# toposware/certificate-stark

Measured on AMD Instinct MI355X. Metric: proofs/sec, state_transition AIR @ 2^20 steps (complete prove(): trace gen, LDE, Blake3 commitments, constraint evaluation, composition, DEEP, FRI, 96 queries), higher is better.
Workload: dtype u64 (63-bit prime field, Montgomery) + u32 (Blake3)

## Files before the change

### certificate-stark_amd/backend.py

```python
import ctypes as C

import numpy as np
import torch

from . import _lib
from ._lib import check, u64p, u8p


def _np_u64(a):
    return np.ascontiguousarray(a, dtype=np.uint64)


def to_numpy_u64(t):
    return t.detach().cpu().contiguous().numpy().view(np.uint64)


class ProofBatch:

    def __init__(self, buf, stride, lens):
        self._buf, self._stride, self._lens = buf, stride, lens

    def __len__(self):
        return len(self._lens)

# ... 22 lines not shown
        self.device = torch.device("cuda", torch.cuda.current_device() if device is None else device)
        torch.cuda.set_device(self.device)
        self.stream = torch.cuda.current_stream(self.device)
        ctx = C.c_void_p()
        check(self.lib.cstark_ctx_create(C.c_int(self.device.index), C.c_void_p(self.stream.cuda_stream), C.byref(ctx)))
        self.ctx = ctx
        self.n_tx = 0
        self.depth = 0
        self.resident = None

    def close(self):
        if getattr(self, "ctx", None):
            self.lib.cstark_ctx_destroy(self.ctx)
            self.ctx = None

    def __del__(self):
        try:
            self.close()
        except Exception:
            pass

    def synchronize(self):
        check(self.lib.cstark_ctx_synchronize(self.ctx))

    def empty_u64(self, *shape):
        return torch.empty(shape, dtype=torch.int64, device=self.device)

    def from_numpy_u64(self, a):
        return torch.from_numpy(_np_u64(a).view(np.int64)).to(self.device)

    @staticmethod
    def _ptr(t, typ=u64p):
        assert t.is_contiguous()
        return C.cast(C.c_void_p(t.data_ptr()), typ)

    def upload_witness(self, w):
        self.resident = None
        s = _lib.TxWitnessStruct()
        s.n_tx, s.merkle_depth = int(w.n_tx), int(w.depth)
        keep = []
        for f, typ in (("initial_roots", u64p), ("final_root", u64p), ("s_old_values", u64p), ("r_old_values", u64p),
                       ("s_indices", u64p), ("r_indices", u64p), ("s_paths", u64p), ("r_paths", u64p),
                       ("deltas", u64p), ("sig_rx", u64p), ("sig_s", u8p)):
            a = np.ascontiguousarray(getattr(w, f), dtype=np.uint8 if typ is u8p else np.uint64)
            keep.append(a)
            setattr(s, f, a.ctypes.data_as(typ))
        check(self.lib.cstark_tx_witness_upload(self.ctx, C.byref(s)))
        self.n_tx, self.depth = int(w.n_tx), int(w.depth)

    def build_trace(self, out=None):
        n = self.n_tx * _lib.TX_CYCLE_LENGTH
        if out is None:
            out = self.empty_u64(_lib.TX_TRACE_WIDTH, n)
        assert out.shape == (_lib.TX_TRACE_WIDTH, n) and out.dtype == torch.int64
        check(self.lib.cstark_tx_build_trace(self.ctx, self._ptr(out)))
        return out

    def field_generator(self):
        self.lib.cstark_field_generator.restype = C.c_uint64
        return int(self.lib.cstark_field_generator())

    def field_lde_offset(self):
        self.lib.cstark_field_lde_offset.restype = C.c_uint64
        return int(self.lib.cstark_field_lde_offset())

    def interpolate_columns(self, evals, out=None):
        width, n = evals.shape
        if out is None:
            out = self.empty_u64(width, n)
        check(self.lib.cstark_interpolate_columns(self.ctx, self._ptr(evals), self._ptr(out), C.c_uint32(width),
                                                  C.c_uint32(n.bit_length() - 1)))
        return out

    def lde_columns(self, coeffs, log_blowup, offset=None, k0=0, nk=None, out=None):
        width, n = coeffs.shape
        nk = (1 << log_blowup) - k0 if nk is None else nk
        if out is None:
            out = self.empty_u64(nk, width, n)
        off = self.field_lde_offset() if offset is None else int(offset)
        check(self.lib.cstark_lde_columns(self.ctx, self._ptr(coeffs), self._ptr(out), C.c_uint32(width),
                                          C.c_uint32(n.bit_length() - 1), C.c_uint32(log_blowup), C.c_uint64(off),
                                          C.c_uint32(k0), C.c_uint32(nk)))
        return out

    def empty_u8(self, *shape):
        return torch.empty(shape, dtype=torch.uint8, device=self.device)

    def hash_rows_fn(self, hash_fn, lde, log_blowup, k0=0):
        nk, width, n = lde.shape
        leaves = self.empty_u8(n << log_blowup, 32)
        check(self.lib.cstark_hash_rows_fn(self.ctx, C.c_uint32(hash_fn), self._ptr(lde), self._ptr(leaves, u8p), C.c_uint32(width),
                                           C.c_uint32(n.bit_length() - 1), C.c_uint32(log_blowup), C.c_uint32(k0), C.c_uint32(nk)))
        return leaves

    def merkle_build_fn(self, hash_fn, nodes):
        check(self.lib.cstark_merkle_build_fn(self.ctx, C.c_uint32(hash_fn), self._ptr(nodes, u8p), C.c_uint32((nodes.shape[0] // 2).bit_length() - 1)))
        return nodes

    def hash_rows(self, lde, log_blowup, k0=0, leaves=None):
        nk, width, n = lde.shape
        if leaves is None:
            leaves = torch.zeros((n << log_blowup, 32), dtype=torch.uint8, device=self.device)
        check(self.lib.cstark_hash_rows(self.ctx, self._ptr(lde), self._ptr(leaves, u8p), C.c_uint32(width),
                                        C.c_uint32(n.bit_length() - 1), C.c_uint32(log_blowup), C.c_uint32(k0), C.c_uint32(nk)))
        return leaves

    def merkle_build(self, nodes):
        L2 = nodes.shape[0]
        check(self.lib.cstark_merkle_build(self.ctx, self._ptr(nodes, u8p), C.c_uint32((L2 // 2).bit_length() - 1)))
        return nodes

    def evaluate_transitions(self, lde, depth, log_blowup=3, k0=0):
        nk, width, n = lde.shape
        out = self.empty_u64(nk, _lib.TX_NUM_CONSTRAINTS, n)
        check(self.lib.cstark_tx_evaluate_transitions(self.ctx, self._ptr(lde), self._ptr(out), C.c_uint32(depth),
                                                      C.c_uint32(n.bit_length() - 1), C.c_uint32(log_blowup), C.c_uint32(k0), C.c_uint32(nk)))
        return out

    def evaluate_constraints(self, lde, coeffs, pub_inputs, depth, log_blowup=3, k0=0, out=None, input_is_lde=False):
        nk, width, n = lde.shape
        if out is None:
            out = self.empty_u64(nk, n)
        pub = (C.c_uint64 * 4)(*[int(v) for v in pub_inputs])
        if input_is_lde:
            assert k0 == 0 and nk == 8 and log_blowup == 3
            check(self.lib.cstark_tx_evaluate_constraints_lde(self.ctx, self._ptr(lde), C.byref(coeffs), pub, self._ptr(out), C.c_uint32(depth),
                                                              C.c_uint32(n.bit_length() - 1)))
            return out
        check(self.lib.cstark_tx_evaluate_constraints(self.ctx, self._ptr(lde), C.byref(coeffs), pub, self._ptr(out), C.c_uint32(depth),
                                                      C.c_uint32(n.bit_length() - 1), C.c_uint32(log_blowup), C.c_uint32(k0), C.c_uint32(nk)))
        return out

    def evaluate_constraints_ext(self, lde, coeff_sets, pub_inputs, depth, log_blowup=3, k0=0, input_is_lde=False):
        nk, width, n = lde.shape
        m = len(coeff_sets)
        out = self.empty_u64(m, nk, n)
        arr = (type(coeff_sets[0]) * m)(*coeff_sets)
        pub = (C.c_uint64 * 4)(*[int(v) for v in pub_inputs])
        if input_is_lde:
            assert k0 == 0 and nk == 8 and log_blowup == 3
            check(self.lib.cstark_tx_evaluate_constraints_ext_lde(self.ctx, self._ptr(lde), arr, C.c_uint32(m), pub, self._ptr(out),
                                                                  C.c_uint32(depth), C.c_uint32(n.bit_length() - 1)))
            return out
        check(self.lib.cstark_tx_evaluate_constraints_ext(self.ctx, self._ptr(lde), arr, C.c_uint32(m), pub, self._ptr(out), C.c_uint32(depth),
                                                          C.c_uint32(n.bit_length() - 1), C.c_uint32(log_blowup), C.c_uint32(k0), C.c_uint32(nk)))
        return out

    AIR_TRANSACTION, AIR_MERKLE, AIR_SCHNORR, AIR_RANGE, AIR_RESCUE_CHAIN = 0, 1, 2, 3, 4

    def rescue_chain_build_trace(self, seed, chain_length):
        s = _np_u64(seed)
        out = self.empty_u64(14, 8 * chain_length)
        check(self.lib.cstark_rescue_chain_build_trace(self.ctx, self._hptr(s), C.c_uint32(chain_length), self._ptr(out)))
        return out

    def rescue_prove(self, options, seed, chain_length):
        s = _np_u64(seed)
        o = self._options_struct(options)
        self.lib.cstark_tx_proof_size_bound.restype = C.c_size_t
        cap = 2 * self.lib.cstark_tx_proof_size_bound(C.c_uint32(max(1, chain_length // 128)), C.byref(o))
        buf = (C.c_uint8 * cap)()
        n = C.c_size_t(0)
        check(self.lib.cstark_rescue_prove(self.ctx, C.byref(o), self._hptr(s), C.c_uint32(chain_length), buf, C.c_size_t(cap), C.byref(n)))
        return bytes(memoryview(buf)[:n.value])

    def merkle_build_trace(self):
# ... 379 lines not shown
```

### certificate-stark_amd/csrc/capi.hip

```cpp
#include <hip/hip_runtime.h>
#include <stdio.h>
#include <stdlib.h>
#include <string.h>
#include <deque>
#include <new>
#include <vector>
#include "../../include/cstark.h"
#include "air_tx_host.h"
#include "blake3.h"
#include "ctx.h"
#include "constraints.h"
#include "deep.h"
#include "ext.h"
#include "hostfield.h"
#include "ntt.h"
#include "trace_gen.h"

namespace cs { thread_local char g_err[512] = ""; }
using cs::fail;
using cs::NttPlan;
using cs::CosetTable;
using cs::PeriodicTable;
using cs::g_err;

// ... 37 lines not shown
    return CSTARK_OK;
}

int get_coset_table(cstark_ctx *c, unsigned log_n, unsigned log_b, uint64_t offset, const CosetTable **out) {
    for (const CosetTable &t : c->cosets)
        if (t.log_n == log_n && t.log_b == log_b && t.offset == offset) { *out = &t; return CSTARK_OK; }
    const size_t n = (size_t)1 << log_n, b = (size_t)1 << log_b;
    CosetTable t{log_n, log_b, offset, nullptr};
    DevGuard g;
    HIP_TRY(g.alloc(&t.s, b * n * 8));
    const uint64_t wbn = cs::host::root_of_unity(log_n + log_b);
    uint64_t shift = offset;
    for (size_t k = 0; k < b; k++) {
        HIP_TRY(cs::ntt_power_table(t.s + k * n, n, shift, c->stream));
        shift = cs::host::mul(shift, wbn);
    }
    cs::NttThreeStepShape shape;
    if (cs::ntt_three_step_shape(log_n, &shape)) {
        const NttPlan *p;
        RC_TRY(get_plan(c, log_n, &p));
        t.aux_words = cs::ntt_aux_coset_words(shape);
        HIP_TRY(g.alloc(&t.aux, b * t.aux_words * 8));
        for (size_t k = 0; k < b; k++) HIP_TRY(cs::ntt_build_aux_coset(t.aux + k * t.aux_words, p->w, t.s + k * n, shape, c->stream));
    }
    c->cosets.push_back(t);
    g.release();
    *out = &c->cosets.back();
    return CSTARK_OK;
}

int ensure_ws(cstark_ctx *c, size_t bytes) {
    if (bytes <= c->ws_bytes) return CSTARK_OK;
    if (c->ws) { HIP_TRY(hipStreamSynchronize(c->stream)); HIP_TRY(hipFree(c->ws)); c->ws = nullptr; c->ws_bytes = 0; }
    HIP_TRY(hipMalloc(&c->ws, bytes));
    c->ws_bytes = bytes;
    return CSTARK_OK;
}

}
int plan_tables(cstark_ctx *c, unsigned log_n, const uint64_t **w, const uint64_t **winv) {
    const NttPlan *p;
    RC_TRY(get_plan(c, log_n, &p));
    *w = p->w; *winv = p->winv;
    return CSTARK_OK;
}
namespace {

int interpolate_impl(cstark_ctx *c, uint64_t *d_evals, uint64_t *d_coeffs, uint32_t width, uint32_t log_n) {
    if (!c || !d_evals || !d_coeffs || width == 0) return fail(CSTARK_ERR_INVALID_ARG, "cstark_interpolate_columns: bad argument");
    if (d_evals == d_coeffs) return fail(CSTARK_ERR_INVALID_ARG, "cstark_interpolate_columns: output must not alias input");
    if (log_n < cs::NTT_MIN_LOG_N || log_n > cs::NTT_MAX_LOG_N) return fail(CSTARK_ERR_UNSUPPORTED, "domain size must be 2^6 .. 2^24");
    HIP_TRY(hipSetDevice(c->device));
    const NttPlan *p;
    RC_TRY(get_plan(c, log_n, &p));
    cs::NttArgs a{};
    a.in = d_evals; a.scratch = d_evals; a.out = d_coeffs;
    a.width = width; a.batch = 1; a.log_n = log_n;
    a.w = p->winv; a.post_scale = p->n_inv; a.do_scale = true; a.inverse = true; a.aux = p->aux_winv;
    HIP_TRY(cs::ntt_columns(a, c->stream));
    return CSTARK_OK;
}

constexpr size_t LDE_EVENT_CAP = 4096;
int lde_mark(cstark_ctx *c) {
    if (c->lde_ev_used == c->lde_ev.size()) {
        if (c->lde_ev.size() >= LDE_EVENT_CAP) return CSTARK_ERR_UNSUPPORTED;

        hipEvent_t e;
        HIP_TRY(hipEventCreate(&e));
        c->lde_ev.push_back(e);
    }
    HIP_TRY(hipEventRecord(c->lde_ev[c->lde_ev_used++], c->stream));
    return CSTARK_OK;
}

const size_t LDE_BATCH_WS_BYTES = [] {
    const char *e = getenv("CSTARK_LDE_BATCH_MB");
    if (!e) return (size_t)7 << 30;
    const long long mb = atoll(e);
    return mb <= 0 ? (size_t)0 : mb > (64ll << 10) ? (size_t)64 << 30 : (size_t)mb << 20;
}();
int lde_impl_inner(cstark_ctx *c, const uint64_t *d_coeffs, uint64_t *d_lde, uint32_t width, uint32_t col0, uint32_t ncols, uint32_t log_n,
                   uint32_t log_blowup, uint64_t domain_offset, uint32_t k0, uint32_t nk);
int lde_impl(cstark_ctx *c, const uint64_t *d_coeffs, uint64_t *d_lde, uint32_t width, uint32_t col0, uint32_t ncols, uint32_t log_n, uint32_t log_blowup,
             uint64_t domain_offset, uint32_t k0, uint32_t nk) {
    bool timed = c && c->part_timing && c->lde_ev_used + 2 <= LDE_EVENT_CAP;
    const size_t mark = timed ? c->lde_ev_used : 0;
    if (timed && lde_mark(c) != CSTARK_OK) { c->lde_ev_used = mark; timed = false; }
    const int rc = lde_impl_inner(c, d_coeffs, d_lde, width, col0, ncols, log_n, log_blowup, domain_offset, k0, nk);
    if (timed) {
        if (rc == CSTARK_OK && lde_mark(c) == CSTARK_OK) c->lde_units += (uint64_t)ncols * nk << log_n;
        else c->lde_ev_used = mark;
    }
    return rc;
}
int lde_impl_inner(cstark_ctx *c, const uint64_t *d_coeffs, uint64_t *d_lde, uint32_t width, uint32_t col0, uint32_t ncols, uint32_t log_n,
                   uint32_t log_blowup, uint64_t domain_offset, uint32_t k0, uint32_t nk) {
    if (!c || !d_coeffs || !d_lde || width == 0 || ncols == 0 || (uint64_t)col0 + ncols > width) return fail(CSTARK_ERR_INVALID_ARG, "cstark_lde_columns: bad argument");
    if (log_n < cs::NTT_MIN_LOG_N || log_n > cs::NTT_MAX_LOG_N || log_blowup > 6) return fail(CSTARK_ERR_UNSUPPORTED, "unsupported domain size");
    if (domain_offset == 0 || domain_offset >= cs::host::P) return fail(CSTARK_ERR_INVALID_ARG, "domain offset must be a nonzero field element");
    if ((uint64_t)k0 + nk > (1ull << log_blowup)) return fail(CSTARK_ERR_INVALID_ARG, "coset range exceeds the blowup factor");
    HIP_TRY(hipSetDevice(c->device));
    const NttPlan *p;
    const CosetTable *t;
    RC_TRY(get_plan(c, log_n, &p));
    RC_TRY(get_coset_table(c, log_n, log_blowup, domain_offset, &t));
    const size_t n = (size_t)1 << log_n;
    RC_TRY(ensure_ws(c, (size_t)width * n * 8));
    cs::NttArgs a{};
    a.in = d_coeffs + (size_t)col0 * n; a.scratch = (uint64_t *)c->ws;
    a.width = ncols; a.log_n = log_n;
    a.w = p->w; a.do_scale = false; a.aux = p->aux_w;
    if (nk > 1 && (size_t)nk * ncols * n * 8 <= LDE_BATCH_WS_BYTES) {
        if (ensure_ws(c, (size_t)nk * ncols * n * 8) == CSTARK_OK) {
            a.scratch = (uint64_t *)c->ws; a.out = d_lde + (size_t)col0 * n; a.batch = nk;
            a.prescale = t->s + (size_t)k0 * n; a.prescale_batch_stride = n;
            a.aux_ps = t->aux ? t->aux + (size_t)k0 * t->aux_words : nullptr; a.aux_ps_batch_stride = t->aux_words;
            a.in_batch_stride = 0; a.scratch_batch_stride = (size_t)ncols * n; a.out_batch_stride = (size_t)width * n;
            HIP_TRY(cs::ntt_columns(a, c->stream));
            return CSTARK_OK;
        }
        (void)hipGetLastError();
        RC_TRY(ensure_ws(c, (size_t)width * n * 8));
        a.scratch = (uint64_t *)c->ws;
    }
    a.batch = 1;
    for (uint32_t k = k0; k < k0 + nk; k++) {
        a.out = d_lde + ((size_t)(k - k0) * width + col0) * n;
        a.prescale = t->s + (size_t)k * n;
        a.aux_ps = t->aux ? t->aux + (size_t)k * t->aux_words : nullptr;
        HIP_TRY(cs::ntt_columns(a, c->stream));
    }
    return CSTARK_OK;
}

int extend_periodic_columns(cstark_ctx *c, const std::vector<uint64_t> &cols, uint32_t ncols, uint32_t log_cycle, unsigned log_n, unsigned log_b,
                            DevGuard &keep, uint64_t **d_tab) {
    const size_t words = (size_t)ncols << log_cycle, n = (size_t)1 << log_n;
    uint64_t *d_cols = nullptr, *d_poly = nullptr;
    DevGuard tmp;
    HIP_TRY(tmp.alloc(&d_cols, words * 8));
    HIP_TRY(tmp.alloc(&d_poly, words * 8));
    HIP_TRY(keep.alloc(d_tab, (words << log_b) * 8));
    HIP_TRY(hipMemcpyAsync(d_cols, cols.data(), words * 8, hipMemcpyHostToDevice, c->stream));
    RC_TRY(interpolate_impl(c, d_cols, d_poly, ncols, log_cycle));
    RC_TRY(lde_impl(c, d_poly, *d_tab, ncols, 0, ncols, log_cycle, log_b, cs::host::pow(cs::host::lde_offset(), n >> log_cycle), 0, 1u << log_b));
    HIP_TRY(hipStreamSynchronize(c->stream));
    return CSTARK_OK;
}

int get_periodic(cstark_ctx *c, unsigned depth, unsigned log_n, unsigned log_b, const PeriodicTable **out) {
    for (const PeriodicTable &t : c->periodic)
        if (t.depth == depth && t.log_n == log_n && t.log_b == log_b) { *out = &t; return CSTARK_OK; }
    if (log_n < 10) return fail(CSTARK_ERR_INVALID_ARG, "the trace must hold at least one 1024-row transaction");
    std::vector<uint64_t> cols;
    if (!cs::host::tx_periodic_columns(depth, cols)) return fail(CSTARK_ERR_INVALID_ARG, "unsupported Merkle depth");
    static_assert(cs::host::TX_CYCLE == 1 << 10, "the cycle of TransactionAir's periodic columns");
    const size_t n = (size_t)1 << log_n, b = (size_t)1 << log_b;
    PeriodicTable t{depth, log_n, log_b, nullptr, nullptr, nullptr};
    DevGuard keep;
    RC_TRY(extend_periodic_columns(c, cols, cs::host::TX_NUM_PERIODIC, 10, log_n, log_b, keep, &t.tab));
    HIP_TRY(keep.alloc(&t.coset, b * cs::CE_COSET_CONSTS * 8));
    const uint64_t g = cs::host::lde_offset();
    std::vector<uint64_t> cc(b * cs::CE_COSET_CONSTS);
    const uint64_t wbn = cs::host::root_of_unity(log_n + log_b);
    uint64_t shift = g;
    for (size_t k = 0; k < b; k++) {
        uint64_t *o = cc.data() + k * cs::CE_COSET_CONSTS;
        o[0] = shift;
        o[1] = cs::host::inv(cs::host::sub(cs::host::pow(shift, n), cs::host::ONE));
        for (int gi = 0; gi < 5; gi++) o[2 + gi] = cs::host::pow(shift, cs::host::tx_group_adjustment(gi, n, n * b));
        o[7] = cs::host::pow(shift, cs::host::tx_boundary_adjustment(n, n * b));
        o[8] = cs::host::pow(shift, n - 1);
        o[9] = 0;
        shift = cs::host::mul(shift, wbn);
    }
    HIP_TRY(hipMemcpyAsync(t.coset, cc.data(), cc.size() * 8, hipMemcpyHostToDevice, c->stream));
    const NttPlan *plan;
    RC_TRY(get_plan(c, log_n, &plan));
    HIP_TRY(keep.alloc(&t.binv, b * 2 * n * 8));
    HIP_TRY(cs::build_boundary_inverses(t.binv, plan->w, t.coset, cs::host::inv(cs::host::root_of_unity(log_n)), log_n, log_b, c->stream));
    HIP_TRY(hipStreamSynchronize(c->stream));
    keep.release();
    c->periodic.push_back(t);
    *out = &c->periodic.back();
    return CSTARK_OK;
}

int get_small_periodic(cstark_ctx *c, int air, unsigned depth, unsigned log_n, unsigned log_b, const PeriodicTable **out) {
    for (const PeriodicTable &t : c->small_periodic)
        if (t.air == air && t.depth == depth && t.log_n == log_n && t.log_b == log_b) { *out = &t; return CSTARK_OK; }
    PeriodicTable t{depth, log_n, log_b, nullptr, nullptr, nullptr, air};
    std::vector<uint64_t> cols;
    DevGuard keep;
    if (air == CSTARK_AIR_MERKLE_UPDATE) {
        if (!cs::host::merkle_periodic_columns(depth, cols)) return fail(CSTARK_ERR_INVALID_ARG, "unsupported Merkle depth");
        RC_TRY(extend_periodic_columns(c, cols, 33, 9, log_n, log_b, keep, &t.tab));
    } else if (air == CSTARK_AIR_SCHNORR) {
        cs::host::schnorr_mask_columns(cols);
        RC_TRY(extend_periodic_columns(c, cols, 36, 9, log_n, log_b, keep, &t.tab));
    } else if (air == CSTARK_AIR_RESCUE_CHAIN) {
        using namespace cs::host;
        rescue_chain_periodic_columns(cols);
        const size_t n = (size_t)1 << log_n, b = (size_t)1 << log_b;
        for (int cidx = 0; cidx < 29; cidx++) intt_small(cols.data() + (size_t)cidx * 8, 3);
        std::vector<uint64_t> tab(b * 29 * 8);
        const uint64_t wbn = root_of_unity(log_n + log_b), w8 = root_of_unity(3);
        uint64_t shift = lde_offset();
        for (size_t k = 0; k < b; k++) {
            uint64_t x = pow(shift, n / 8);
            for (int m = 0; m < 8; m++) {
                for (int cidx = 0; cidx < 29; cidx++) {
                    const uint64_t *co = cols.data() + (size_t)cidx * 8;
                    uint64_t v = 0;
                    for (int d = 7; d >= 0; d--) v = add(mul(v, x), co[d]);
                    tab[(k * 29 + cidx) * 8 + m] = v;
// ... 18 lines not shown
              uint32_t nk, cs::CeParams *p) {
    if (!c || !d_lde || !d_out) return fail(CSTARK_ERR_INVALID_ARG, "constraint evaluation: null argument");
    if (((uintptr_t)d_lde & 15) != 0) return fail(CSTARK_ERR_INVALID_ARG, "constraint evaluation: d_lde must be 16-byte aligned (16-byte LDS-DMA pieces)");
    if (log_n < 10 || log_n > cs::NTT_MAX_LOG_N) return fail(CSTARK_ERR_INVALID_ARG, "trace length must be 2^10 .. 2^24");
    if (log_blowup != 3) return fail(CSTARK_ERR_UNSUPPORTED, "TransactionAir needs a constraint-evaluation blowup of 8 (max degree 7, src/air.rs:76-108)");
    if ((uint64_t)k0 + nk > (1ull << log_blowup) || nk == 0) return fail(CSTARK_ERR_INVALID_ARG, "coset range exceeds the blowup factor");
    HIP_TRY(hipSetDevice(c->device));
    const PeriodicTable *pt;
    const NttPlan *plan;
    RC_TRY(get_periodic(c, merkle_depth, log_n, log_blowup, &pt));
    RC_TRY(get_plan(c, log_n, &plan));
    const uint64_t n = 1ull << log_n, ce = n << log_blowup;
    *p = cs::CeParams{};
    p->lde = d_lde; p->ptab = pt->tab; p->w = plan->w; p->coset = pt->coset; p->binv = pt->binv; p->out = d_out;
    p->w_last = cs::host::inv(cs::host::root_of_unity(log_n));
    for (int g = 0; g < 5; g++) p->adj_mod_n[g] = (uint32_t)(cs::host::tx_group_adjustment(g, n, ce) & (n - 1));
    p->badj_mod_n = (uint32_t)(cs::host::tx_boundary_adjustment(n, ce) & (n - 1));
    p->log_n = log_n; p->log_b = log_blowup; p->k0 = k0;
    return CSTARK_OK;
}

}

extern "C" {

const char *cstark_last_error(void) { return g_err; }
const char *cstark_version(void) { return "certificate-stark_amd 0.2 (gfx950)"; }

int cstark_ctx_create(int device, void *stream, cstark_ctx **out) {
    if (!out) return fail(CSTARK_ERR_INVALID_ARG, "cstark_ctx_create: out is null");
    int count = 0;
    if (hipGetDeviceCount(&count) != hipSuccess || count == 0)
        return fail(CSTARK_ERR_NO_DEVICE, "no HIP device visible (this backend has no CPU fallback)");
    if (device < 0) HIP_TRY(hipGetDevice(&device));
    if (device >= count) return fail(CSTARK_ERR_INVALID_ARG, "device index out of range");
    HIP_TRY(hipSetDevice(device));
    cstark_ctx *c = new (std::nothrow) cstark_ctx();
    if (!c) return fail(CSTARK_ERR_OOM, "host allocation failed");
    c->device = device;
    c->stream = (hipStream_t)stream;
    int prio_lo = 0, prio_hi = 0;
    (void)hipDeviceGetStreamPriorityRange(&prio_lo, &prio_hi);
    if (hipStreamCreateWithPriority(&c->side, hipStreamNonBlocking, prio_hi) != hipSuccess ||
        hipStreamCreateWithPriority(&c->side2, hipStreamNonBlocking, prio_hi) != hipSuccess ||
        hipEventCreateWithFlags(&c->ev_fork, hipEventDisableTiming) != hipSuccess || hipEventCreateWithFlags(&c->ev_join, hipEventDisableTiming) != hipSuccess ||
        hipEventCreateWithFlags(&c->ev_join2, hipEventDisableTiming) != hipSuccess || hipEventCreateWithFlags(&c->ev_mid, hipEventDisableTiming) != hipSuccess) {
        delete c;
        return fail(CSTARK_ERR_HIP, "could not create the internal stream / events");
    }
    *out = c;
    return CSTARK_OK;
}
int cstark_ctx_create_own_stream(int device, cstark_ctx **out) {
    if (!out) return fail(CSTARK_ERR_INVALID_ARG, "cstark_ctx_create_own_stream: out is null");
    RC_TRY(cstark_ctx_create(device, nullptr, out));
    cstark_ctx *c = *out;
    if (hipStreamCreateWithFlags(&c->stream, hipStreamNonBlocking) != hipSuccess) {
        c->stream = nullptr;
        cstark_ctx_destroy(c);
        *out = nullptr;
        return fail(CSTARK_ERR_HIP, "could not create the context's stream");
    }
    c->owns_stream = true;
    return CSTARK_OK;
}

void cstark_ctx_destroy(cstark_ctx *c) {
    if (!c) return;
    (void)hipSetDevice(c->device);
    (void)hipStreamSynchronize(c->stream);
    if (c->side) { (void)hipStreamSynchronize(c->side); (void)hipStreamDestroy(c->side); }
    if (c->side2) { (void)hipStreamSynchronize(c->side2); (void)hipStreamDestroy(c->side2); }
    if (c->ev_join2) (void)hipEventDestroy(c->ev_join2);
    if (c->ev_mid) (void)hipEventDestroy(c->ev_mid);
    if (c->ev_fork) (void)hipEventDestroy(c->ev_fork);
    if (c->ev_join) (void)hipEventDestroy(c->ev_join);
    if (c->wit_buf) (void)hipFree(c->wit_buf);
    if (c->ws) (void)hipFree(c->ws);
    if (c->coef_buf) (void)hipFree(c->coef_buf);
    if (c->coef_stage) (void)hipHostFree(c->coef_stage);
    if (c->coef_ev) (void)hipEventDestroy(c->coef_ev);
    for (NttPlan &p : c->plans) { (void)hipFree(p.w); (void)hipFree(p.winv); (void)hipFree(p.aux_w); (void)hipFree(p.aux_winv); }
    for (CosetTable &t : c->cosets) { (void)hipFree(t.s); (void)hipFree(t.aux); }
    for (PeriodicTable &t : c->periodic) { (void)hipFree(t.tab); (void)hipFree(t.coset); (void)hipFree(t.binv); }
    for (PeriodicTable &t : c->small_periodic) (void)hipFree(t.tab);
    for (cs::AssertInverseTable &t : c->assert_inv) (void)hipFree(t.tab);
    for (cs::AirCombineStatic &t : c->air_static) (void)hipFree(t.d_static);
    if (c->air_coef_buf) (void)hipFree(c->air_coef_buf);
    if (c->air_coef_stage) (void)hipHostFree(c->air_coef_stage);
    if (c->air_coef_ev) (void)hipEventDestroy(c->air_coef_ev);
    if (c->deep_buf) (void)hipFree(c->deep_buf);
    if (c->deep_stage) (void)hipHostFree(c->deep_stage);
    if (c->deep_ev) (void)hipEventDestroy(c->deep_ev);
    if (c->desc_buf) (void)hipFree(c->desc_buf);
    if (c->rb_dev) (void)hipFree(c->rb_dev);
    if (c->shard_bit37) (void)hipFree(c->shard_bit37);
    if (c->rb_host) (void)hipHostFree(c->rb_host);
    if (c->tail_buf) (void)hipFree(c->tail_buf);
    if (c->arena) cs::prove_arena_free(c->arena);
    if (c->verify) cs::verify_arena_free(c->verify);
    for (hipEvent_t e : c->part_ev) if (e) (void)hipEventDestroy(e);
    for (hipEvent_t e : c->lde_ev) (void)hipEventDestroy(e);
    if (c->owns_stream && c->stream) (void)hipStreamDestroy(c->stream);
    delete c;
}

int cstark_ctx_synchronize(cstark_ctx *c) {
    if (!c) return fail(CSTARK_ERR_INVALID_ARG, "null context");
    HIP_TRY(hipStreamSynchronize(c->stream));
    return CSTARK_OK;
}

int cstark_malloc(cstark_ctx *c, size_t bytes, void **d_ptr) {
    if (!c || !d_ptr) return fail(CSTARK_ERR_INVALID_ARG, "cstark_malloc: null argument");
    HIP_TRY(hipSetDevice(c->device));
    HIP_TRY(hipMalloc(d_ptr, bytes));
    return CSTARK_OK;
}
int cstark_free(cstark_ctx *c, void *d_ptr) {
    if (!c) return fail(CSTARK_ERR_INVALID_ARG, "null context");
    HIP_TRY(hipSetDevice(c->device));
    HIP_TRY(hipStreamSynchronize(c->stream));
    HIP_TRY(hipFree(d_ptr));
    return CSTARK_OK;
}
int cstark_memcpy_h2d(cstark_ctx *c, void *d_dst, const void *src, size_t bytes) {
    if (!c || (!d_dst && bytes) || (!src && bytes)) return fail(CSTARK_ERR_INVALID_ARG, "cstark_memcpy_h2d: null argument");
    HIP_TRY(hipMemcpyAsync(d_dst, src, bytes, hipMemcpyHostToDevice, c->stream));
    HIP_TRY(hipStreamSynchronize(c->stream));
    return CSTARK_OK;
}
int cstark_memcpy_d2h(cstark_ctx *c, void *dst, const void *d_src, size_t bytes) {
    if (!c || (!dst && bytes) || (!d_src && bytes)) return fail(CSTARK_ERR_INVALID_ARG, "cstark_memcpy_d2h: null argument");
    HIP_TRY(hipMemcpyAsync(dst, d_src, bytes, hipMemcpyDeviceToHost, c->stream));
    HIP_TRY(hipStreamSynchronize(c->stream));
    return CSTARK_OK;
}

int cstark_tx_witness_upload(cstark_ctx *c, const cstark_tx_witness *w) {
    if (!c || !w) return fail(CSTARK_ERR_INVALID_ARG, "cstark_tx_witness_upload: null argument");
    const size_t n = w->n_tx, d = w->merkle_depth;
    if (n == 0) return fail(CSTARK_ERR_INVALID_ARG, "n_tx must be positive");
    if (d == 0 || ((d + 1) & d) != 0 || 8 * d + 7 > 511) return fail(CSTARK_ERR_INVALID_ARG, "tree depth must be one less than a power of 2 and at most 31");
    if (!w->initial_roots || !w->s_old_values || !w->r_old_values || !w->s_indices || !w->r_indices || !w->s_paths || !w->r_paths ||
        !w->deltas || !w->sig_rx || !w->sig_s)
        return fail(CSTARK_ERR_INVALID_ARG, "witness array pointer is null");
    HIP_TRY(hipSetDevice(c->device));
    const size_t sz[] = {n * 7 * 8, n * 14 * 8, n * 14 * 8, n * 8, n * 8, n * (d + 1) * 7 * 8, n * (d + 1) * 7 * 8, n * 8, n * 6 * 8, n * 4 * 8, n * 32};
    const void *src[] = {w->initial_roots, w->s_old_values, w->r_old_values, w->s_indices, w->r_indices, w->s_paths, w->r_paths, w->deltas, w->sig_rx, nullptr, w->sig_s};
    size_t off[12] = {0};
    for (int i = 0; i < 11; i++) off[i + 1] = off[i] + ((sz[i] + 255) & ~(size_t)255);
    if (off[11] > c->wit_bytes) {
        if (c->wit_buf) { HIP_TRY(hipStreamSynchronize(c->stream)); HIP_TRY(hipFree(c->wit_buf)); c->wit_buf = nullptr; c->wit_bytes = 0; }
        HIP_TRY(hipMalloc(&c->wit_buf, off[11]));
        c->wit_bytes = off[11];
    }
    char *base = (char *)c->wit_buf;
    for (int i = 0; i < 11; i++)
        if (src[i]) HIP_TRY(hipMemcpyAsync(base + off[i], src[i], sz[i], hipMemcpyHostToDevice, c->stream));
    HIP_TRY(hipStreamSynchronize(c->stream));
    cs::TxWitnessDev &dv = c->wit;
    dv.n_tx = (uint32_t)n;
    dv.depth = (uint32_t)d;
    dv.initial_roots = (const uint64_t *)(base + off[0]);
    dv.s_old = (const uint64_t *)(base + off[1]);
    dv.r_old = (const uint64_t *)(base + off[2]);
    dv.s_idx = (const uint64_t *)(base + off[3]);
    dv.r_idx = (const uint64_t *)(base + off[4]);
    dv.s_paths = (const uint64_t *)(base + off[5]);
    dv.r_paths = (const uint64_t *)(base + off[6]);
    dv.deltas = (const uint64_t *)(base + off[7]);
    dv.sig_rx = (const uint64_t *)(base + off[8]);
    dv.h_limbs = (uint64_t *)(base + off[9]);
    dv.sig_s = (const uint8_t *)(base + off[10]);
    dv.msg_tail = nullptr;
    return CSTARK_OK;
}

int cstark_tx_build_trace(cstark_ctx *c, uint64_t *d_trace) {
    if (!c || !d_trace) return fail(CSTARK_ERR_INVALID_ARG, "cstark_tx_build_trace: null argument");
    if (!c->wit_buf || c->wit.n_tx == 0) return fail(CSTARK_ERR_INVALID_ARG, "no witness uploaded");
    HIP_TRY(hipSetDevice(c->device));
    HIP_TRY(cs::launch_trace_gen(c->wit, d_trace, c->stream, c->side, c->ev_fork, c->ev_join));
    return CSTARK_OK;
}

uint64_t cstark_field_generator(void) { return cs::host::generator(); }
uint64_t cstark_field_lde_offset(void) { return cs::host::lde_offset(); }
uint64_t cstark_field_root_of_unity(uint32_t log_n) { return log_n <= 55 ? cs::host::root_of_unity(log_n) : 0; }

int cstark_interpolate_columns(cstark_ctx *c, uint64_t *d_evals, uint64_t *d_coeffs, uint32_t width, uint32_t log_n) {
    return interpolate_impl(c, d_evals, d_coeffs, width, log_n);
}
int cstark_lde_columns(cstark_ctx *c, const uint64_t *d_coeffs, uint64_t *d_lde, uint32_t width, uint32_t log_n, uint32_t log_blowup,
                       uint64_t domain_offset, uint32_t k0, uint32_t nk) {
    return lde_impl(c, d_coeffs, d_lde, width, 0, width, log_n, log_blowup, domain_offset, k0, nk);
}

int cstark_composition_columns(cstark_ctx *c, const uint64_t *d_combined, uint64_t *d_cols, uint32_t log_n, uint32_t log_blowup) {
    if (!c || !d_combined || !d_cols) return fail(CSTARK_ERR_INVALID_ARG, "cstark_composition_columns: null argument");
    if (log_n < cs::NTT_MIN_LOG_N || log_n + log_blowup > cs::NTT_MAX_LOG_N || log_blowup == 0 || log_blowup > 6)
        return fail(CSTARK_ERR_UNSUPPORTED, "composition domain must be 2^7 .. 2^24 points");
    HIP_TRY(hipSetDevice(c->device));
    const size_t N = (size_t)1 << (log_n + log_blowup);
    RC_TRY(ensure_ws(c, 2 * N * 8));
    uint64_t *nat = (uint64_t *)c->ws, *h = nat + N;
    if (log_blowup <= 3) {
        const NttPlan *pn, *pN;
        RC_TRY(get_plan(c, log_n, &pn));
        RC_TRY(get_plan(c, log_n + log_blowup, &pN));
        cs::NttArgs a{};
        a.in = d_combined; a.scratch = h; a.out = nat; a.width = 1u << log_blowup; a.batch = 1; a.log_n = log_n;
        a.w = pn->winv; a.post_scale = pn->n_inv; a.do_scale = true; a.inverse = true; a.aux = pn->aux_winv;
        HIP_TRY(cs::ntt_columns(a, c->stream));
        const uint64_t b_inv = cs::host::inv(cs::host::from_u64(1ull << log_blowup));
        HIP_TRY(cs::coset_combine(nat, h, log_n, log_blowup, pN->winv, b_inv, c->stream));
        HIP_TRY(cs::split_columns(h, d_cols, log_n, log_blowup, cs::host::inv(cs::host::lde_offset()), c->stream));
        return CSTARK_OK;
    }
    HIP_TRY(cs::interleave_cosets(d_combined, nat, log_n, log_blowup, c->stream));
    const NttPlan *p;
    RC_TRY(get_plan(c, log_n + log_blowup, &p));
    cs::NttArgs a{};
    a.in = nat; a.scratch = nat; a.out = h; a.width = 1; a.batch = 1; a.log_n = log_n + log_blowup;
    a.w = p->winv; a.post_scale = p->n_inv; a.do_scale = true; a.inverse = true; a.aux = p->aux_winv;
    HIP_TRY(cs::ntt_columns(a, c->stream));
    HIP_TRY(cs::split_columns(h, d_cols, log_n, log_blowup, cs::host::inv(cs::host::lde_offset()), c->stream));
    return CSTARK_OK;
}

int cstark_evaluate_polys_at(cstark_ctx *c, const uint64_t *d_coeffs, uint32_t width, uint32_t log_n, const uint64_t *points, uint32_t npts,
                             uint64_t *out ) {
    if (!c || !d_coeffs || !points || !out || width == 0 || npts == 0 || npts > 16) return fail(CSTARK_ERR_INVALID_ARG, "cstark_evaluate_polys_at: bad argument");
    if (log_n > 30) return fail(CSTARK_ERR_INVALID_ARG, "bad polynomial size");
    HIP_TRY(hipSetDevice(c->device));
    const size_t need = ((size_t)npts + (size_t)npts * width + cs::poly_eval_scratch_words(width, log_n, npts)) * 8;
    if (need > c->desc_bytes) {
        if (c->desc_buf) { HIP_TRY(hipStreamSynchronize(c->stream)); HIP_TRY(hipFree(c->desc_buf)); c->desc_buf = nullptr; c->desc_bytes = 0; }
        HIP_TRY(hipMalloc(&c->desc_buf, need));
        c->desc_bytes = need;
    }
    uint64_t *d_pts = (uint64_t *)c->desc_buf, *d_out = d_pts + npts, *d_scr = d_out + (size_t)npts * width;
    HIP_TRY(hipMemcpyAsync(d_pts, points, (size_t)npts * 8, hipMemcpyHostToDevice, c->stream));
    HIP_TRY(cs::poly_eval(d_coeffs, width, log_n, d_pts, npts, d_out, d_scr, c->stream));
    HIP_TRY(hipMemcpyAsync(out, d_out, (size_t)npts * width * 8, hipMemcpyDeviceToHost, c->stream));
    HIP_TRY(cs::stream_wait(c->stream));
    return CSTARK_OK;
}

int cstark_deep_composition(cstark_ctx *c, const uint64_t *d_trace_lde, const uint64_t *d_comp_lde, uint32_t width, uint32_t n_comp,
                            uint64_t z, const uint64_t *ood_trace, const uint64_t *ood_comp, const uint64_t *alpha, const uint64_t *beta,
                            const uint64_t *delta, uint64_t deg_a, uint64_t deg_b, uint64_t *d_out, uint32_t log_n, uint32_t log_blowup,
                            uint32_t k0, uint32_t nk) {
    if (!c || !d_trace_lde || !d_comp_lde || !ood_trace || !ood_comp || !alpha || !beta || !delta || !d_out || nk == 0 || width == 0 || n_comp == 0)
        return fail(CSTARK_ERR_INVALID_ARG, "cstark_deep_composition: bad argument");
    if (log_n < cs::NTT_MIN_LOG_N || log_n > cs::NTT_MAX_LOG_N || log_blowup > 6 || (uint64_t)k0 + nk > (1ull << log_blowup)) return fail(CSTARK_ERR_INVALID_ARG, "bad domain parameters");
    HIP_TRY(hipSetDevice(c->device));
    const NttPlan *plan;
    RC_TRY(get_plan(c, log_n, &plan));
    const size_t b = (size_t)1 << log_blowup, nco = 2 * (size_t)width + n_comp, words = 2 * nco + b;
    if (c->deep_words < words) {
        HIP_TRY(hipStreamSynchronize(c->stream));
        if (c->deep_buf) { HIP_TRY(hipFree(c->deep_buf)); c->deep_buf = nullptr; }
        if (c->deep_stage) { HIP_TRY(hipHostFree(c->deep_stage)); c->deep_stage = nullptr; }
        c->deep_words = 0;
        HIP_TRY(hipMalloc((void **)&c->deep_buf, words * 8));
        HIP_TRY(hipHostMalloc((void **)&c->deep_stage, words * 8, hipHostMallocDefault));
        if (!c->deep_ev) HIP_TRY(hipEventCreateWithFlags(&c->deep_ev, hipEventDisableTiming));
        c->deep_words = words;
    } else {
        HIP_TRY(hipEventSynchronize(c->deep_ev));
    }
    uint64_t *blk = c->deep_stage;
    memcpy(blk, alpha, width * 8); memcpy(blk + width, beta, width * 8); memcpy(blk + 2 * width, delta, n_comp * 8);
    memcpy(blk + nco, ood_trace, 2 * (size_t)width * 8); memcpy(blk + nco + 2 * width, ood_comp, n_comp * 8);
    const uint64_t wbn = cs::host::root_of_unity(log_n + log_blowup);
    uint64_t shift = cs::host::lde_offset();
    for (size_t k = 0; k < b; k++) { blk[2 * nco + k] = shift; shift = cs::host::mul(shift, wbn); }
    HIP_TRY(hipMemcpyAsync(c->deep_buf, blk, words * 8, hipMemcpyHostToDevice, c->stream));
    HIP_TRY(hipEventRecord(c->deep_ev, c->stream));
// ... 223 lines not shown
                                       log_blowup, 1u << log_blowup);
}
int cstark_fri_fold4_ext(cstark_ctx *c, const uint64_t *d_evals, uint64_t *d_out, uint32_t log_n, uint64_t domain_offset, uint32_t m, const uint64_t *alpha) {
    if (!c || !d_evals || !d_out || !alpha || d_evals == d_out || (m != 2 && m != 3)) return fail(CSTARK_ERR_INVALID_ARG, "cstark_fri_fold4_ext: bad argument");
    if (log_n < cs::NTT_MIN_LOG_N || log_n > cs::NTT_MAX_LOG_N) return fail(CSTARK_ERR_UNSUPPORTED, "layer size must be 2^6 .. 2^24");
    if (domain_offset == 0 || domain_offset >= cs::host::P) return fail(CSTARK_ERR_INVALID_ARG, "offset must be a nonzero field element");
    for (uint32_t i = 0; i < m; i++) if (alpha[i] >= cs::host::P) return fail(CSTARK_ERR_INVALID_ARG, "alpha is not an extension element");
    HIP_TRY(hipSetDevice(c->device));
    const NttPlan *p;
    RC_TRY(get_plan(c, log_n, &p));
    HIP_TRY(cs::fri_fold4_ext(d_evals, d_out, log_n, p->winv, cs::host::inv(domain_offset), alpha, m, cs::host::inv(cs::host::from_u64(4)), c->stream));
    return CSTARK_OK;
}
int cstark_fri_fold_ext(cstark_ctx *c, const uint64_t *d_evals, uint64_t *d_out, uint32_t log_n, uint32_t folding_factor, uint64_t domain_offset, uint32_t m,
                        const uint64_t *alpha) {
    if (!c || !d_evals || !d_out || !alpha || d_evals == d_out || (m != 2 && m != 3)) return fail(CSTARK_ERR_INVALID_ARG, "cstark_fri_fold_ext: bad argument");
    if (folding_factor != 4 && folding_factor != 8 && folding_factor != 16) return fail(CSTARK_ERR_UNSUPPORTED, "FRI folding factor must be 4, 8 or 16");
    if (log_n < cs::NTT_MIN_LOG_N || log_n > cs::NTT_MAX_LOG_N) return fail(CSTARK_ERR_UNSUPPORTED, "layer size must be 2^6 .. 2^24");
    if (domain_offset == 0 || domain_offset >= cs::host::P) return fail(CSTARK_ERR_INVALID_ARG, "offset must be a nonzero field element");
    for (uint32_t i = 0; i < m; i++) if (alpha[i] >= cs::host::P) return fail(CSTARK_ERR_INVALID_ARG, "alpha is not an extension element");
    HIP_TRY(hipSetDevice(c->device));
    const NttPlan *p;
    RC_TRY(get_plan(c, log_n, &p));
    const unsigned log_f = folding_factor == 4 ? 2 : folding_factor == 8 ? 3 : 4;
    HIP_TRY(cs::fri_fold_ext(d_evals, d_out, log_n, log_f, p->winv, cs::host::inv(domain_offset), alpha, m, cs::host::inv(cs::host::from_u64(folding_factor)), c->stream));
    return CSTARK_OK;
}

int cstark_hash_rows(cstark_ctx *c, const uint64_t *d_lde, uint8_t *d_leaves, uint32_t width, uint32_t log_n, uint32_t log_blowup,
                     uint32_t k0, uint32_t nk) {
    if (!c || !d_lde || !d_leaves) return fail(CSTARK_ERR_INVALID_ARG, "cstark_hash_rows: null argument");
    if (width == 0 || width > 128) return fail(CSTARK_ERR_UNSUPPORTED, "row width must be 1..128 elements (single Blake3 chunk)");
    if (log_n > 30 || log_blowup > 6 || (uint64_t)k0 + nk > (1ull << log_blowup)) return fail(CSTARK_ERR_INVALID_ARG, "bad domain parameters");
    if (((uintptr_t)d_leaves & 15) != 0) return fail(CSTARK_ERR_INVALID_ARG, "d_leaves must be 16-byte aligned");
    HIP_TRY(hipSetDevice(c->device));
    HIP_TRY(cs::hash_rows(d_lde, d_leaves, width, log_n, log_blowup, k0, nk, c->stream));
    return CSTARK_OK;
}

int cstark_hash_rows_fn(cstark_ctx *c, uint32_t hash_fn, const uint64_t *d_lde, uint8_t *d_leaves, uint32_t width, uint32_t log_n, uint32_t log_blowup,
                        uint32_t k0, uint32_t nk) {
    if (hash_fn == 0) return cstark_hash_rows(c, d_lde, d_leaves, width, log_n, log_blowup, k0, nk);
    if (hash_fn != 1) return fail(CSTARK_ERR_UNSUPPORTED, "hash_fn must be 0 (Blake3_256) or 1 (Sha3_256)");
    if (!c || !d_lde || !d_leaves) return fail(CSTARK_ERR_INVALID_ARG, "cstark_hash_rows_fn: null argument");
    if (width == 0 || width > 128) return fail(CSTARK_ERR_UNSUPPORTED, "row width must be 1..128 elements");
    if (log_n > 30 || log_blowup > 6 || (uint64_t)k0 + nk > (1ull << log_blowup)) return fail(CSTARK_ERR_INVALID_ARG, "bad domain parameters");
    if (((uintptr_t)d_leaves & 15) != 0) return fail(CSTARK_ERR_INVALID_ARG, "d_leaves must be 16-byte aligned");
    HIP_TRY(hipSetDevice(c->device));
    HIP_TRY(cs::hash_rows_sha3(d_lde, d_leaves, width, log_n, log_blowup, k0, nk, c->stream));
    return CSTARK_OK;
}
int cstark_merkle_build_fn(cstark_ctx *c, uint32_t hash_fn, uint8_t *d_nodes, uint32_t log_leaves) {
    if (hash_fn == 0) return cstark_merkle_build(c, d_nodes, log_leaves);
    if (hash_fn != 1) return fail(CSTARK_ERR_UNSUPPORTED, "hash_fn must be 0 (Blake3_256) or 1 (Sha3_256)");
    if (!c || !d_nodes) return fail(CSTARK_ERR_INVALID_ARG, "cstark_merkle_build_fn: null argument");
    if (log_leaves == 0 || log_leaves > 30) return fail(CSTARK_ERR_INVALID_ARG, "tree must have 2 .. 2^30 leaves");
    if (((uintptr_t)d_nodes & 15) != 0) return fail(CSTARK_ERR_INVALID_ARG, "d_nodes must be 16-byte aligned");
    HIP_TRY(hipSetDevice(c->device));
    HIP_TRY(cs::merkle_build_sha3(d_nodes, log_leaves, c->stream));
    return CSTARK_OK;
}

int cstark_merkle_build(cstark_ctx *c, uint8_t *d_nodes, uint32_t log_leaves) {
    if (!c || !d_nodes) return fail(CSTARK_ERR_INVALID_ARG, "cstark_merkle_build: null argument");
    if (log_leaves == 0 || log_leaves > 30) return fail(CSTARK_ERR_INVALID_ARG, "tree must have 2 .. 2^30 leaves");
    if (((uintptr_t)d_nodes & 15) != 0) return fail(CSTARK_ERR_INVALID_ARG, "d_nodes must be 16-byte aligned");
    HIP_TRY(hipSetDevice(c->device));
    HIP_TRY(cs::merkle_build(d_nodes, log_leaves, c->stream));
    return CSTARK_OK;
}

int cstark_tx_evaluate_transitions(cstark_ctx *c, const uint64_t *d_lde, uint64_t *d_out, uint32_t merkle_depth, uint32_t log_n,
                                   uint32_t log_blowup, uint32_t k0, uint32_t nk) {
    cs::CeParams p;
    RC_TRY(ce_params(c, d_lde, d_out, merkle_depth, log_n, log_blowup, k0, nk, &p));
    HIP_TRY(cs::launch_eval_transitions(p, nk, c->stream));
    return CSTARK_OK;
}

}
int lde_column_range(cstark_ctx *c, const uint64_t *d_coeffs, uint64_t *d_lde, uint32_t width, uint32_t col0, uint32_t ncols, uint32_t log_n,
                     uint32_t log_blowup, uint64_t domain_offset, uint32_t k0, uint32_t nk) {
    return lde_impl(c, d_coeffs, d_lde, width, col0, ncols, log_n, log_blowup, domain_offset, k0, nk);
}
int tx_build_trace_split(cstark_ctx *c, uint64_t *d_trace) {
    if (!c || !d_trace) return fail(CSTARK_ERR_INVALID_ARG, "tx_build_trace_split: null argument");
    if (!c->wit_buf || c->wit.n_tx == 0) return fail(CSTARK_ERR_INVALID_ARG, "no witness uploaded");
    HIP_TRY(hipSetDevice(c->device));
    HIP_TRY(cs::launch_trace_gen_split(c->wit, d_trace, c->stream, c->side, c->side2, c->ev_fork, c->ev_join, c->ev_mid, c->ev_join2));
    return CSTARK_OK;
}
static constexpr size_t TX_COEF_WORDS = (size_t)cs::CE_MAX_SETS * cs::CE_COEF_WORDS;
static int ensure_coef_buf(cstark_ctx *c) {
    static_assert(sizeof(cstark_tx_coeffs) == cs::CE_COEF_WORDS * 8, "coefficient block layout");
    if (!c->coef_buf) HIP_TRY(hipMalloc((void **)&c->coef_buf, (TX_COEF_WORDS + (size_t)cs::CE_MAX_SETS * cs::CE_RTAB_WORDS) * 8));
    return CSTARK_OK;
}
int tx_coef_device_block(cstark_ctx *c, uint64_t **d_coef) {
    HIP_TRY(hipSetDevice(c->device));
    RC_TRY(ensure_coef_buf(c));
    *d_coef = c->coef_buf;
    return CSTARK_OK;
}
static int upload_coeffs(cstark_ctx *c, const cstark_tx_coeffs *coeffs, uint32_t m, cs::CeParams &p) {
    constexpr size_t COEF_WORDS = TX_COEF_WORDS;
    RC_TRY(ensure_coef_buf(c));
    if (!c->coef_stage) {
        if (!c->coef_ev) HIP_TRY(hipEventCreateWithFlags(&c->coef_ev, hipEventDisableTiming));
        HIP_TRY(hipHostMalloc(&c->coef_stage, (size_t)cs::CE_MAX_SETS * sizeof(cstark_tx_coeffs), hipHostMallocDefault));
    } else {
        HIP_TRY(hipEventSynchronize(c->coef_ev));
    }
    memcpy(c->coef_stage, coeffs, (size_t)m * sizeof(cstark_tx_coeffs));
    HIP_TRY(hipMemcpyAsync(c->coef_buf, c->coef_stage, (size_t)m * sizeof(cstark_tx_coeffs), hipMemcpyHostToDevice, c->stream));
    HIP_TRY(hipEventRecord(c->coef_ev, c->stream));
    p.coef = c->coef_buf;
    p.rtab = c->coef_buf + COEF_WORDS;
    p.m = m;
    return CSTARK_OK;
}

struct SplitMerge { unsigned log_n = 0; cs::CosetMergeDesc desc; cs::CosetMergeTerm hi; };
static const SplitMerge &tx_split_merge(unsigned log_n) {
    static thread_local SplitMerge sm;
    if (sm.log_n == log_n) return sm;
    const uint64_t n = 1ull << log_n, g = cs::host::lde_offset();
    uint64_t adj[3];
    for (int i = 0; i < 3; i++) adj[i] = cs::host::tx_group_adjustment(i, n, 8 * n);
    static const int first[cs::CE_SPLIT_FAMILIES] = {0, cs::CE_SPLIT_FAM0, 7, 9, 11}, count[cs::CE_SPLIT_FAMILIES] = {4, 3, 2, 2, 2};
    sm.desc = cs::CosetMergeDesc{};
    sm.desc.families = cs::CE_SPLIT_FAMILIES;
    sm.desc.tables_per_set = cs::CE_SPLIT_TABLES;
    sm.desc.raw_family = cs::CE_SPLIT_FAMILIES - 1;
    for (int f = 0; f < cs::CE_SPLIT_FAMILIES; f++) {
        sm.desc.terms[f] = count[f];
        for (int t = 0; t < count[f]; t++) sm.desc.term[f][t] = cs::coset_merge_term(first[f] + t, t ? adj[t - 1] : 0, log_n, g);
    }
    sm.hi = cs::coset_merge_term(0, adj[0], log_n, cs::host::mul(g, cs::host::root_of_unity(log_n + 3)), 2);
    sm.log_n = log_n;
    return sm;
}

namespace {

struct SplitStage {
    unsigned log_n;
    size_t n;
    const NttPlan *pn, *p4, *p8;
    const CosetTable *t1;
    hipStream_t stream;
};
int split_stage(cstark_ctx *c, unsigned log_n, SplitStage *s) {
    *s = SplitStage{log_n, (size_t)1 << log_n, nullptr, nullptr, nullptr, nullptr, c->stream};
    RC_TRY(get_plan(c, log_n, &s->pn));
    RC_TRY(get_plan(c, log_n + 2, &s->p4));
    RC_TRY(get_plan(c, log_n + 3, &s->p8));
    return get_coset_table(c, log_n, 3, cs::host::from_u64(1), &s->t1);
}

int inverse_columns(const SplitStage &s, const uint64_t *in, uint64_t *scratch, uint64_t *out, unsigned width, unsigned batch = 1, size_t batch_stride = 0) {
    cs::NttArgs a{};
    a.in = in; a.scratch = scratch; a.out = out; a.width = width; a.batch = batch; a.log_n = s.log_n;
    a.in_batch_stride = batch_stride; a.scratch_batch_stride = batch_stride; a.out_batch_stride = batch_stride;
    a.w = s.pn->winv; a.post_scale = s.pn->n_inv; a.do_scale = true; a.inverse = true; a.aux = s.pn->aux_winv;
    HIP_TRY(cs::ntt_columns(a, s.stream));
    return CSTARK_OK;
// ... 668 lines not shown
```

### certificate-stark_amd/csrc/ctx.h

```cpp
#pragma once
#include <stdlib.h>
#include <hip/hip_runtime.h>
#include <stdio.h>
#include <deque>
#include <vector>
#include "../../include/cstark.h"
#include "constraints.h"
#include "trace_gen.h"

#include <chrono>
namespace cs {
inline hipError_t stream_wait(hipStream_t st) {
    static const bool block = [] { const char *e = getenv("CSTARK_SYNC_BLOCK"); return e && atoi(e) != 0; }();
    static const long spin_us = [] { const char *e = getenv("CSTARK_SPIN_US"); return e ? atol(e) : 200L; }();
    if (block || spin_us <= 0) return hipStreamSynchronize(st);
    const auto t0 = std::chrono::steady_clock::now();
    hipError_t e;
    for (unsigned it = 0; (e = hipStreamQuery(st)) == hipErrorNotReady; it++) {
#if defined(__x86_64__) || defined(__i386__)
        __builtin_ia32_pause();
#endif
        if ((it & 15) == 15 && std::chrono::duration_cast<std::chrono::microseconds>(std::chrono::steady_clock::now() - t0).count() > spin_us)
            return hipStreamSynchronize(st);
    }
    return e;
}
inline hipError_t stream_wait_tail(hipStream_t st, hipEvent_t near_end) {
    static const bool block = [] { const char *e = getenv("CSTARK_SYNC_BLOCK"); return e && atoi(e) != 0; }();
    if (block) return hipStreamSynchronize(st);
    hipError_t e = hipEventSynchronize(near_end);
    if (e != hipSuccess) return e;
    const auto t0 = std::chrono::steady_clock::now();
    for (unsigned it = 0; (e = hipStreamQuery(st)) == hipErrorNotReady; it++) {
#if defined(__x86_64__) || defined(__i386__)
        __builtin_ia32_pause();
#endif
        if ((it & 15) == 15 && std::chrono::duration_cast<std::chrono::microseconds>(std::chrono::steady_clock::now() - t0).count() > 5000)
            return hipStreamSynchronize(st);
    }
    return e;
}
}

namespace cs {

extern thread_local char g_err[512];

inline int fail(int code, const char *fmt, const char *detail = "") {
    snprintf(g_err, sizeof g_err, fmt, detail);
    return code;
}
#define HIP_TRY(expr)                                                                                                              \
    do {                                                                                                                           \
        hipError_t e_ = (expr);                                                                                                    \
        if (e_ != hipSuccess) return cs::fail(e_ == hipErrorOutOfMemory ? CSTARK_ERR_OOM : CSTARK_ERR_HIP, #expr ": %s", hipGetErrorString(e_)); \
    } while (0)
#define RC_TRY(expr)            \
    do {                        \
        int rc_ = (expr);       \
        if (rc_) return rc_;    \
    } while (0)

struct NttPlan {
    unsigned log_n;
    uint64_t *w, *winv;
    uint64_t n_inv;
    uint64_t *aux_w = nullptr, *aux_winv = nullptr;
};
struct CosetTable {
    unsigned log_n, log_b;
    uint64_t offset;
    uint64_t *s;
    uint64_t *aux = nullptr;
    size_t aux_words = 0;
};
struct PeriodicTable {
    unsigned depth, log_n, log_b;
    uint64_t *tab;
    uint64_t *coset;
    uint64_t *binv;
    int air = 0;
};
struct AssertInverseTable {
    unsigned log_n, log_b;
    uint64_t m, zc;
    uint64_t *tab;
};
struct AirCombineStatic {
    int air;
    uint32_t n_items, log_n, log_b;
    AirCombineParams p;
    std::vector<uint32_t> t_grp;
    uint64_t *d_static;
};
enum class AirTransitions {
    Materialised,
    MerkleFused,
    SchnorrFused,
};
struct AirStageRequest {
    int air = 0;
    uint32_t n_items = 0;
    uint32_t log_n = 0, log_blowup = 0, k0 = 0, nk = 0;
    const uint64_t *d_lde = nullptr;
    uint64_t *d_out = nullptr;
    AirTransitions source = AirTransitions::Materialised;
    const uint64_t *d_evals = nullptr;
    uint32_t merkle_depth = 0;
    const uint64_t *d_aux_lde = nullptr;
    bool own_extension = false;
    const uint64_t *t_alpha = nullptr, *t_beta = nullptr, *b_alpha = nullptr, *b_beta = nullptr, *assertion_values = nullptr;
    const uint64_t *d_coefs = nullptr, *d_avalues = nullptr;
    const uint64_t *d_avals_lde = nullptr;
    uint32_t n_avals = 0;
};
struct ProveArena;
void prove_arena_free(ProveArena *a);
struct VerifyArena;
void verify_arena_free(VerifyArena *a);

}

struct cstark_ctx {
    int device = 0;
    hipStream_t stream = nullptr;
    bool owns_stream = false;
    hipStream_t side = nullptr, side2 = nullptr;
    hipEvent_t ev_fork = nullptr, ev_join = nullptr, ev_join2 = nullptr, ev_mid = nullptr;
    void *wit_buf = nullptr;
    size_t wit_bytes = 0;
    cs::TxWitnessDev wit{};
    std::deque<cs::NttPlan> plans;
    std::deque<cs::CosetTable> cosets;
    std::deque<cs::PeriodicTable> periodic;
    uint64_t *coef_buf = nullptr;
    void *coef_stage = nullptr;
    hipEvent_t coef_ev = nullptr;
    std::deque<cs::AssertInverseTable> assert_inv;
    std::deque<cs::AirCombineStatic> air_static;
    uint64_t *air_coef_buf = nullptr, *air_coef_stage = nullptr;
    size_t air_coef_words = 0;
    hipEvent_t air_coef_ev = nullptr;
    uint64_t *deep_buf = nullptr, *deep_stage = nullptr;
    size_t deep_words = 0;
    hipEvent_t deep_ev = nullptr;
    std::deque<cs::PeriodicTable> small_periodic;
    void *desc_buf = nullptr;
    hipEvent_t part_ev[cs::CE_NUM_PARTS + 1] = {};
    bool part_timing = false, part_valid = false;
    std::vector<hipEvent_t> lde_ev;
    size_t lde_ev_used = 0;
    uint64_t lde_units = 0;
    uint64_t *tail_buf = nullptr;
    std::vector<uint64_t> schnorr_rx;
    std::vector<uint64_t> schnorr_av_stage;
    std::vector<uint64_t> schnorr_pub;
    std::vector<uint8_t> schnorr_s;
    uint8_t schnorr_seed[32] = {}, schnorr_seed_key[12] = {};
    size_t tail_bytes = 0;
    size_t desc_bytes = 0;
    cs::ProveArena *arena = nullptr;
    cs::VerifyArena *verify = nullptr;
    void *ws = nullptr;
    size_t ws_bytes = 0;
    uint64_t *shard_bit37 = nullptr;
    size_t shard_bit37_words = 0;
    void *rb_dev = nullptr, *rb_host = nullptr;
    size_t rb_dev_bytes = 0, rb_host_bytes = 0;
};
int fri_coin_fold_dev(cstark_ctx *c, uint32_t *d_seed, const uint8_t *d_root, uint64_t *d_alpha, uint32_t *d_root_out, const uint64_t *d_evals,
                      uint64_t *d_out, uint32_t log_n, uint32_t log_f, uint64_t domain_offset, uint32_t m);
int hash_rows_slots(cstark_ctx *c, uint32_t hash_fn, const uint64_t *d_lde, uint8_t *d_leaves, uint32_t width, uint32_t log_n, uint32_t log_blowup, uint32_t log_s);
int plan_tables(cstark_ctx *c, unsigned log_n, const uint64_t **w, const uint64_t **winv);

struct cstark_tx_coeffs;
int tx_evaluate_constraints_sets(cstark_ctx *c, const uint64_t *d_lde, const cstark_tx_coeffs *coeffs, uint32_t m, const uint64_t pub_inputs[4],
                                 uint64_t *const *d_outs, uint32_t merkle_depth, uint32_t log_n, uint32_t log_blowup, uint32_t k0, uint32_t nk,
                                 bool input_is_lde, const uint64_t *d_pub = nullptr);
int tx_coef_device_block(cstark_ctx *c, uint64_t **d_coef);
int air_stage(cstark_ctx *c, const cs::AirStageRequest &rq);
int tx_evaluate_constraints_shard(cstark_ctx *c, const uint64_t *d_lde, const uint64_t *d_coeffs, const cstark_tx_coeffs *coeffs, const uint64_t pub_inputs[4],
                                  uint64_t *d_out, uint32_t merkle_depth, uint32_t log_n, uint32_t k0, uint32_t nk);
int tx_shard_combine(cstark_ctx *c, const uint64_t *d_parts, uint64_t *d_out, uint32_t log_n, uint32_t nk);
constexpr uint32_t TX_LATE_COLS = 37;
constexpr uint32_t TX_COPY_COLS = 65;
int tx_build_trace_split(cstark_ctx *c, uint64_t *d_trace);
int lde_column_range(cstark_ctx *c, const uint64_t *d_coeffs, uint64_t *d_lde, uint32_t width, uint32_t col0, uint32_t ncols, uint32_t log_n,
                     uint32_t log_blowup, uint64_t domain_offset, uint32_t k0, uint32_t nk);
int evaluate_ood_frames(cstark_ctx *c, const uint64_t *d_coeffs, uint32_t width, const uint64_t *d_ccoef, uint32_t n_comp, uint32_t log_n,
                        const uint64_t zpts[2], uint64_t zb, uint64_t *out_trace, uint64_t *out_comp);
int ood_frames_dev(cstark_ctx *c, const uint64_t *d_coeffs, uint32_t width, const uint64_t *d_ccoef, uint32_t n_comp, uint32_t log_n, const uint64_t *d_pts,
                   uint64_t *d_out);
int desc_reserve(cstark_ctx *c, size_t bytes);
size_t ood_frames_dev_scratch_bytes(uint32_t width, uint32_t n_comp, uint32_t log_n, uint32_t m);
int ood_frames_dev_ext(cstark_ctx *c, const uint64_t *d_coeffs, uint32_t width, const uint64_t *d_ccoef, uint32_t n_comp, uint32_t log_n, uint32_t m,
                       const uint64_t *d_pts, uint64_t *d_out);
int deep_composition_ext_dev(cstark_ctx *c, const uint64_t *d_trace_lde, const uint64_t *d_comp_lde, uint32_t width, uint32_t n_comp, uint32_t m,
                             const uint64_t *d_coef, const uint64_t *d_ood, uint64_t *d_scal, const uint64_t *d_shifts, uint64_t *d_out, uint32_t log_n,
                             uint32_t log_blowup, uint32_t nk);
int deep_composition_ext_cosets(cstark_ctx *c, const uint64_t *d_trace_lde, const uint64_t *d_comp_lde, uint32_t width, uint32_t n_comp, uint32_t m,
                                const uint64_t *z, const uint64_t *ood_trace, const uint64_t *ood_comp, const uint64_t *alpha, const uint64_t *beta,
                                const uint64_t *delta, const uint64_t *deg_a, const uint64_t *deg_b, uint64_t *d_out, uint32_t log_n, uint32_t log_blowup,
                                uint32_t nk);
```

### certificate-stark_amd/csrc/ntt.h

```cpp
#pragma once
#include <hip/hip_runtime.h>
#include <stddef.h>
#include <stdint.h>

namespace cs {

constexpr unsigned NTT_MIN_LOG_N = 6, NTT_MAX_LOG_N = 24;

struct NttArgs {
    const uint64_t *in;
    uint64_t *scratch;
    uint64_t *out;
    unsigned width, batch, log_n;
    const uint64_t *w;
    const uint64_t *prescale;
    size_t prescale_batch_stride;
    uint64_t post_scale;
    bool do_scale;
    bool inverse;
    size_t in_batch_stride, scratch_batch_stride, out_batch_stride;
    const uint64_t *aux = nullptr, *aux_ps = nullptr;
    size_t aux_ps_batch_stride = 0;
};

struct NttThreeStepShape { unsigned log_r, log_c, log_kb; };
bool ntt_three_step_shape(unsigned log_n, NttThreeStepShape *s);
size_t ntt_aux_plan_words(const NttThreeStepShape &s);
size_t ntt_aux_coset_words(const NttThreeStepShape &s);
hipError_t ntt_build_aux_plan(uint64_t *d_aux, const uint64_t *d_w, const NttThreeStepShape &s, hipStream_t stream);
hipError_t ntt_build_aux_coset(uint64_t *d_aux, const uint64_t *d_w, const uint64_t *d_s, const NttThreeStepShape &s, hipStream_t stream);

hipError_t ntt_columns(const NttArgs &a, hipStream_t stream);
hipError_t ntt_power_table(uint64_t *d_table, size_t n, uint64_t base, hipStream_t stream);

hipError_t interleave_cosets(const uint64_t *d_in, uint64_t *d_out, unsigned log_n, unsigned log_b, hipStream_t stream);
hipError_t coset_combine(const uint64_t *d_b, uint64_t *d_h, unsigned log_n, unsigned log_b, const uint64_t *d_winv_N, uint64_t b_inv,
                         hipStream_t stream, unsigned tables = 1);
hipError_t coset_even_to_odd(const uint64_t *d_b, uint64_t *d_out, unsigned log_n, unsigned tables, const uint64_t *d_winv_4n, const uint64_t *d_w_8n,
                             uint64_t quarter, hipStream_t stream, unsigned kc0 = 0, unsigned nkc = 4);
struct CosetMergeTerm {
    uint32_t table, r;
    uint64_t c[4][2];
};
constexpr int COSET_MERGE_MAX_FAMILIES = 5, COSET_MERGE_MAX_TERMS = 4;
struct CosetMergeDesc {
    uint32_t families, tables_per_set;
    uint32_t terms[COSET_MERGE_MAX_FAMILIES];
    CosetMergeTerm term[COSET_MERGE_MAX_FAMILIES][COSET_MERGE_MAX_TERMS];
    int32_t raw_family;
};
CosetMergeTerm coset_merge_term(unsigned table, uint64_t e, unsigned log_n, uint64_t base, unsigned k0 = 1);
hipError_t coset_even_to_odd_merged(const uint64_t *d_b, uint64_t *d_out, unsigned log_n, unsigned sets, const CosetMergeDesc &desc,
                                    const uint64_t *d_winv_4n, const uint64_t *d_w_8n, uint64_t quarter, uint64_t *d_raw, hipStream_t stream);
hipError_t split_columns(const uint64_t *d_h, uint64_t *d_out, unsigned log_n, unsigned log_b, uint64_t ginv, hipStream_t stream);

}
```

### certificate-stark_amd/csrc/ntt.hip

```cpp
#include "ntt.h"
#include "fp.cuh"
#include "hostfield.h"
#include "../../include/cstark_conventions.h"
#ifdef CS_NTT_NOMATH
#define fp_mul(a, b) ((a) ^ (b))
#define fp_add(a, b) ((a) + (b))
#define fp_sub(a, b) ((a) - (b))
#define fp_sub_lazy(a, b) ((a) - (b))
#endif
#ifndef CS_NTT_SKIP
#define CS_NTT_SKIP 0
#endif

namespace cs {
namespace {

__device__ __forceinline__ fp mb_load(const fp *row, unsigned lane_off, unsigned fake) { return (CS_NTT_SKIP & 16) ? (fp)fake : row[lane_off]; }
__device__ __forceinline__ void mb_store(fp *row, unsigned lane_off, fp val) {
    if (!(CS_NTT_SKIP & 8) || val == 0x123456789abcdefull) row[lane_off] = val;
}
constexpr bool MB_NO_TWIDDLE_FILL = (CS_NTT_SKIP & 1) != 0, MB_NO_PRESCALE = (CS_NTT_SKIP & 2) != 0, MB_NO_OUTPUT_FACTOR = (CS_NTT_SKIP & 4) != 0;

constexpr int NT = 256;

// ... 121 lines not shown
            }
        }
    }
}
__host__ __device__ constexpr unsigned cx_brev(unsigned x, int bits) {
    unsigned r = 0;
    for (int i = 0; i < bits; i++) r |= ((x >> i) & 1u) << (bits - 1 - i);
    return r;
}

constexpr int L2 = 8;
__device__ __forceinline__ unsigned xcd_pair_tile(unsigned y) { return (y & ~15u) | ((y & 7u) << 1) | ((y >> 3) & 1u); }

template <int LA, int LB, int LC>
struct V4 {
    static constexpr int A = 1 << LA, Bn = 1 << LB, Cn = 1 << LC, T = Bn * Cn, M = A * T, LOGM = LA + LB + LC;
    static constexpr int NT = L2 * T;
    static constexpr int J2 = A / Bn;
    static constexpr int J3 = A / Cn;
    static_assert(LA >= LB && LB >= LC && LC >= 1, "step sizes must not increase");
};

template <int LA, int LB, int LC>
__device__ __forceinline__ void fill_twiddles(fp *tw, const fp *__restrict__ tab) {
    using G = V4<LA, LB, LC>;
    if (MB_NO_TWIDDLE_FILL) { for (unsigned e = threadIdx.x; e < G::M; e += G::NT) tw[e] = e; }
    else for (unsigned e = threadIdx.x; e < G::M; e += G::NT) tw[e] = tab[e];
}

struct ColsTables { const fp *ps_row, *outf, *ratio; };
template <int LA, int LB, int LC>
__device__ __forceinline__ ColsTables cols_tables(const fp *__restrict__ aux, const fp *__restrict__ aux_ps, size_t aux_ps_batch_stride, unsigned bz,
                                                  unsigned log_c) {
    constexpr int M = V4<LA, LB, LC>::M;
    ColsTables tb;
    tb.ps_row = aux_ps ? aux_ps + bz * aux_ps_batch_stride : nullptr;
    tb.outf = tb.ps_row ? tb.ps_row + M : aux + M + ((size_t)2 << log_c);
    tb.ratio = aux + M + ((size_t)1 << log_c);
    return tb;
}

template <int LA, int LB, int LC>
__device__ __forceinline__ void cols_load_prescaled(fp (&a)[1 << LA], const fp *__restrict__ src, const fp *__restrict__ ps_row, unsigned log_c, unsigned t,
                                                    unsigned c) {
    constexpr int A = V4<LA, LB, LC>::A, T = V4<LA, LB, LC>::T;
    const unsigned lane_off = (t << log_c) + c;
#pragma unroll
    for (int r1 = 0; r1 < A; r1++) a[r1] = mb_load(src + ((size_t)(r1 * T) << log_c), lane_off, lane_off + r1);
    if (!MB_NO_PRESCALE && ps_row) {
#pragma unroll
        for (int r1 = 0; r1 < A; r1++) a[r1] = fp_mul(a[r1], ps_row[r1 * T + t]);
    }
}

template <int LA, int LB, int LC>
__device__ __forceinline__ void cols_store_task(const fp (&x)[1 << LC], unsigned kb, unsigned c, unsigned log_c, const ColsTables &tb, fp *__restrict__ dst) {
    constexpr int A = V4<LA, LB, LC>::A, Bn = V4<LA, LB, LC>::Bn, Cn = V4<LA, LB, LC>::Cn;
    fp g, ratio;
    if (MB_NO_OUTPUT_FACTOR) { g = kb + c; ratio = c; }
    else { g = tb.outf[((size_t)kb << log_c) + c]; ratio = tb.ratio[c]; }
    const unsigned lane_off = (kb << log_c) + c;
#pragma unroll
    for (int k3 = 0; k3 < Cn; k3++) {
        fp *row = dst + ((size_t)(A * Bn * k3) << log_c);
        const fp val = fp_mul(x[cx_brev(k3, LC)], g);
        mb_store(row, lane_off, val);
        if (k3 + 1 < Cn) g = fp_mul(g, ratio);
    }
}

template <int LA, int LB, int LC>
__device__ __forceinline__ void rows_store_task(const fp (&x)[1 << LC], unsigned kb, unsigned l, unsigned log_r, fp post_scale, int do_scale,
                                                fp *__restrict__ dst_tile) {
    constexpr int A = V4<LA, LB, LC>::A, Bn = V4<LA, LB, LC>::Bn, Cn = V4<LA, LB, LC>::Cn;
    const unsigned out_lane = (kb << log_r) + l;
#pragma unroll
    for (int p = 0; p < Cn; p++) {
        fp val = x[p];
        if (do_scale) val = fp_mul(val, post_scale);
        mb_store(dst_tile + ((size_t)(A * Bn * cx_brev(p, LC)) << log_r), out_lane, val);
    }
}

constexpr int V4_TILES = 1;


template <int LA, int LB, int LC, bool INV>
__device__ __forceinline__ void cols_v4_finish(fp *tile, const fp *tw, const fp *__restrict__ w, const fp *__restrict__ ps, fp *__restrict__ dst,
                                               unsigned log_c, unsigned c, unsigned t, unsigned l, const fp *__restrict__ outf,
                                               const fp *__restrict__ ratio_tab) {
    using G = V4<LA, LB, LC>;
    constexpr int A = G::A, Bn = G::Bn, Cn = G::Cn, T = G::T;
    fp z[G::J2][Bn];
#pragma unroll
    for (int j = 0; j < G::J2; j++) {
        const unsigned u = t + T * j, k1 = u / Cn, r3 = u % Cn;
#pragma unroll
        for (int r2 = 0; r2 < Bn; r2++) z[j][r2] = tile[((size_t)k1 * T + r2 * Cn + r3) * L2 + l];
    }
    __syncthreads();
#pragma unroll
    for (int j = 0; j < G::J2; j++) {
        const unsigned u = t + T * j, k1 = u / Cn, r3 = u % Cn;
        reg_ntt_dif<LB, INV>(z[j]);
#pragma unroll
        for (int p = 0; p < Bn; p++) {
            const unsigned k2 = cx_brev(p, LB);
            const fp v = (k2 == 0) ? z[j][p] : fp_mul(z[j][p], tw[(A * k2) * r3]);
            tile[((size_t)k1 * T + k2 * Cn + (r3 ^ (k2 % Cn))) * L2 + l] = v;
        }
    }
    __syncthreads();
#pragma unroll
    for (int j = 0; j < G::J3; j++) {
        const unsigned v = t + T * j, k1 = v / Bn, k2 = v % Bn;
        fp x[Cn];
#pragma unroll
        for (int r3 = 0; r3 < Cn; r3++) x[r3] = tile[((size_t)k1 * T + k2 * Cn + (r3 ^ (k2 % Cn))) * L2 + l];
        reg_ntt_dif<LC, INV>(x);
        const unsigned kb = k1 + A * k2;
        fp g, ratio;
        if (MB_NO_OUTPUT_FACTOR) { g = kb + c; ratio = c; }
        else if (outf) {
            g = outf[((size_t)kb << log_c) + c];
            ratio = ratio_tab[c];
        } else {
            g = w[(size_t)kb * c];
            if (ps) g = fp_mul(g, ps[c]);
            ratio = w[(size_t)(A * Bn) * c];
        }
        const unsigned lane_off = (kb << log_c) + c;
#pragma unroll
        for (int k3 = 0; k3 < Cn; k3++) {
            fp *row = dst + ((size_t)(A * Bn * k3) << log_c);
            const fp val = fp_mul(x[cx_brev(k3, LC)], g);
            mb_store(row, lane_off, val);
            if (k3 + 1 < Cn) g = fp_mul(g, ratio);
        }
    }
}

template <int LA, int LB, int LC, bool INV>
__global__ __launch_bounds__((V4<LA, LB, LC>::NT), 4) void k_ntt_cols_v4(const fp *__restrict__ in, fp *__restrict__ out, unsigned log_n,
                                                                        const fp *__restrict__ w, const fp *__restrict__ prescale,
                                                                        size_t in_batch_stride, size_t out_batch_stride, size_t prescale_batch_stride,
                                                                        const fp *__restrict__ aux, const fp *__restrict__ aux_ps,
                                                                        size_t aux_ps_batch_stride) {
    using G = V4<LA, LB, LC>;
    constexpr int A = G::A, T = G::T, M = G::M, LOGM = G::LOGM;
    extern __shared__ __attribute__((aligned(16))) fp smem[];
    fp *tile = smem;
    fp *tw = smem + (size_t)M * L2;
    const unsigned log_c = log_n - LOGM;
    const size_t n = (size_t)1 << log_n;
    const unsigned bz = blockIdx.y, tile_id = blockIdx.x;
    const fp *src = in + bz * in_batch_stride + (size_t)blockIdx.z * n;
    fp *dst = out + bz * out_batch_stride + (size_t)blockIdx.z * n;
    const fp *ps = prescale ? prescale + bz * prescale_batch_stride : nullptr;
    const unsigned l = threadIdx.x % L2, t = threadIdx.x / L2;
    const fp *ps_row = (ps && aux_ps) ? aux_ps + bz * aux_ps_batch_stride : nullptr;
    const fp *outf = !aux ? nullptr : ps ? (ps_row ? ps_row + M : nullptr) : aux + M + ((size_t)2 << log_c);
    const fp *ratio_tab = aux ? aux + M + ((size_t)1 << log_c) : nullptr;

    if (MB_NO_TWIDDLE_FILL) { for (unsigned e = threadIdx.x; e < M; e += G::NT) tw[e] = e; }
    else if (aux) for (unsigned e = threadIdx.x; e < M; e += G::NT) tw[e] = aux[e];
    else for (unsigned e = threadIdx.x; e < M; e += G::NT) tw[e] = w[(size_t)e << log_c];
// ... 44 lines not shown
                                                                        const fp *__restrict__ w, fp post_scale, int do_scale,
                                                                        size_t in_batch_stride, size_t out_batch_stride, const fp *__restrict__ aux_tw) {
    using G = V4<LA, LB, LC>;
    constexpr int A = G::A, Bn = G::Bn, Cn = G::Cn, T = G::T, M = G::M, LOGM = G::LOGM;
    constexpr int TP = T + 4;
    extern __shared__ __attribute__((aligned(16))) fp smem[];
    fp *tile = smem;
    fp *tw = smem + (size_t)A * L2 * TP;
    const unsigned log_r = log_n - LOGM;
    const size_t n = (size_t)1 << log_n;
    const fp *src = in + blockIdx.x * in_batch_stride + (size_t)blockIdx.z * n;
    fp *dst = out + blockIdx.x * out_batch_stride + (size_t)blockIdx.z * n;
    const unsigned s1 = threadIdx.x % T, l1 = threadIdx.x / T;
    const unsigned l = threadIdx.x % L2, t = threadIdx.x / L2;

    if (MB_NO_TWIDDLE_FILL) { for (unsigned e = threadIdx.x; e < M; e += G::NT) tw[e] = e; }
    else if (aux_tw) for (unsigned e = threadIdx.x; e < M; e += G::NT) tw[e] = aux_tw[e];
    else for (unsigned e = threadIdx.x; e < M; e += G::NT) tw[e] = w[(size_t)e << log_r];
    fp nxt[A];
    const unsigned in_lane = (l1 << LOGM) + s1;
    {
        const unsigned k10 = xcd_pair_tile(blockIdx.y * V4_TILES) * L2;
#pragma unroll
        for (int c1 = 0; c1 < A; c1++) nxt[c1] = mb_load(src + ((size_t)k10 << LOGM) + c1 * T, in_lane, in_lane + c1);
    }
    __syncthreads();
#pragma unroll 1
    for (int it = 0; it < V4_TILES; it++) {
        const unsigned k10 = xcd_pair_tile(blockIdx.y * V4_TILES + it) * L2;
        {
            fp a[A];
#pragma unroll
            for (int c1 = 0; c1 < A; c1++) a[c1] = nxt[c1];
            if (it + 1 < V4_TILES) {
                const unsigned k11 = xcd_pair_tile(blockIdx.y * V4_TILES + it + 1) * L2;
#pragma unroll
                for (int c1 = 0; c1 < A; c1++) nxt[c1] = (src + ((size_t)k11 << LOGM) + c1 * T)[in_lane];
            }
            __builtin_amdgcn_sched_barrier(0);
            reg_ntt_dif<LA, INV>(a);
#pragma unroll
            for (int p = 0; p < A; p++) {
                const unsigned j1 = cx_brev(p, LA);
                tile[((size_t)j1 * L2 + l1) * TP + s1] = (j1 == 0) ? a[p] : fp_mul(a[p], tw[j1 * s1]);
            }
        }
        __syncthreads();
        fp z[G::J2][Bn];
#pragma unroll
        for (int j = 0; j < G::J2; j++) {
            const unsigned u = t + T * j, j1 = u / Cn, c3 = u % Cn;
#pragma unroll
            for (int c2 = 0; c2 < Bn; c2++) z[j][c2] = tile[((size_t)j1 * L2 + l) * TP + c2 * Cn + c3];
        }
        __syncthreads();
#pragma unroll
        for (int j = 0; j < G::J2; j++) {
            const unsigned u = t + T * j, j1 = u / Cn, c3 = u % Cn;
            reg_ntt_dif<LB, INV>(z[j]);
#pragma unroll
            for (int p = 0; p < Bn; p++) {
                const unsigned j2 = cx_brev(p, LB);
                const fp v = (j2 == 0) ? z[j][p] : fp_mul(z[j][p], tw[(A * j2) * c3]);
                tile[((size_t)j1 * L2 + l) * TP + j2 * Cn + (c3 ^ (j2 % Cn))] = v;
            }
        }
        __syncthreads();
#pragma unroll
        for (int j = 0; j < G::J3; j++) {
            const unsigned v = t + T * j, j1 = v / Bn, j2 = v % Bn;
            fp x[Cn];
#pragma unroll
            for (int c3 = 0; c3 < Cn; c3++) x[c3] = tile[((size_t)j1 * L2 + l) * TP + j2 * Cn + (c3 ^ (j2 % Cn))];
            reg_ntt_dif<LC, INV>(x);
            const unsigned out_lane = ((j1 + A * j2) << log_r) + l;
#pragma unroll
            for (int p = 0; p < Cn; p++) {
                fp val = x[p];
                if (do_scale) val = fp_mul(val, post_scale);
                mb_store(dst + ((size_t)(A * Bn * cx_brev(p, LC)) << log_r) + k10, out_lane, val);
            }
        }
        __syncthreads();
    }
}

constexpr int V5_COLS_WAVES = 5;
constexpr int V5_ROWS_WAVES = 6;
template <int LA, int LB, int LC, bool INV>
__global__ __launch_bounds__((V4<LA, LB, LC>::NT), V5_COLS_WAVES) void k_ntt_cols_v5(const fp *__restrict__ in, fp *__restrict__ out, unsigned log_n,
                                                                                    size_t in_batch_stride, size_t out_batch_stride,
                                                                                    const fp *__restrict__ aux, const fp *__restrict__ aux_ps,
                                                                                    size_t aux_ps_batch_stride) {
    using G = V4<LA, LB, LC>;
    constexpr int A = G::A, Bn = G::Bn, Cn = G::Cn, T = G::T, M = G::M, LOGM = G::LOGM, AH = A / 2;
    static_assert(G::J2 == 2 && G::J3 == 2 && Bn == AH && Cn == AH, "two tasks per thread and step, one per half");
    extern __shared__ __attribute__((aligned(16))) fp smem[];
    fp *tile = smem;
    fp *tw = smem + (size_t)(M / 2) * L2;
    const unsigned log_c = log_n - LOGM;
    const size_t n = (size_t)1 << log_n;
    const unsigned bz = blockIdx.y;
    const fp *src = in + bz * in_batch_stride + (size_t)blockIdx.z * n;
    fp *dst = out + bz * out_batch_stride + (size_t)blockIdx.z * n;
    const unsigned l = threadIdx.x % L2, t = threadIdx.x / L2;
    const ColsTables tb = cols_tables<LA, LB, LC>(aux, aux_ps, aux_ps_batch_stride, bz, log_c);
    const unsigned c = xcd_pair_tile(blockIdx.x) * L2 + l;

    fill_twiddles<LA, LB, LC>(tw, aux);
    fp a[A];
    cols_load_prescaled<LA, LB, LC>(a, src, tb.ps_row, log_c, t, c);
    reg_ntt_dif<LA, INV>(a);
    __syncthreads();
    const unsigned kh = t / Cn, r3 = t % Cn;
    fp z[2][Bn];
#pragma unroll
    for (int h = 0; h < 2; h++) {
#pragma unroll
        for (int p = 0; p < A; p++) {
            const unsigned k1 = cx_brev(p, LA);
            if ((int)(k1 / AH) == h) tile[((size_t)(k1 % AH) * T + t) * L2 + l] = (k1 == 0) ? a[p] : fp_mul(a[p], tw[k1 * t]);
        }
        __syncthreads();
#pragma unroll
        for (int r2 = 0; r2 < Bn; r2++) z[h][r2] = tile[((size_t)kh * T + r2 * Cn + r3) * L2 + l];
        __syncthreads();
    }
    const unsigned k1s = t / Bn, k2 = t % Bn;
#pragma unroll
    for (int h = 0; h < 2; h++) {
        reg_ntt_dif<LB, INV>(z[h]);
#pragma unroll
        for (int p = 0; p < Bn; p++) {
            const unsigned j2 = cx_brev(p, LB);
            const fp v = (j2 == 0) ? z[h][p] : fp_mul(z[h][p], tw[(A * j2) * r3]);
            tile[((size_t)kh * T + j2 * Cn + (r3 ^ (j2 % Cn))) * L2 + l] = v;
        }
        __syncthreads();
        fp x[Cn];
#pragma unroll
        for (int q = 0; q < Cn; q++) x[q] = tile[((size_t)k1s * T + k2 * Cn + (q ^ (k2 % Cn))) * L2 + l];
        if (h == 0) __syncthreads();
        reg_ntt_dif<LC, INV>(x);
        cols_store_task<LA, LB, LC>(x, (k1s + AH * h) + A * k2, c, log_c, tb, dst);
    }
}

template <int LA, int LB, int LC, bool INV>
__global__ __launch_bounds__((V4<LA, LB, LC>::NT), V5_ROWS_WAVES) void k_ntt_rows_v5(const fp *__restrict__ in, fp *__restrict__ out, unsigned log_n,
                                                                                    fp post_scale, int do_scale, size_t in_batch_stride,
                                                                                    size_t out_batch_stride, const fp *__restrict__ aux_tw) {
    using G = V4<LA, LB, LC>;
    constexpr int A = G::A, Bn = G::Bn, Cn = G::Cn, T = G::T, LOGM = G::LOGM, AH = A / 2;
    static_assert(G::J2 == 2 && G::J3 == 2 && Bn == AH && Cn == AH, "two tasks per thread and step, one per half");
    constexpr int TP = T + 4;
    extern __shared__ __attribute__((aligned(16))) fp smem[];
    fp *tile = smem;
    fp *tw = smem + (size_t)AH * L2 * TP;
    const unsigned log_r = log_n - LOGM;
    const size_t n = (size_t)1 << log_n;
    const fp *src = in + blockIdx.x * in_batch_stride + (size_t)blockIdx.z * n;
    fp *dst = out + blockIdx.x * out_batch_stride + (size_t)blockIdx.z * n;
    const unsigned s1 = threadIdx.x % T, l1 = threadIdx.x / T;
    const unsigned l = threadIdx.x % L2, t = threadIdx.x / L2;
    const unsigned k10 = xcd_pair_tile(blockIdx.y) * L2;
    fp a[A];
    const unsigned in_lane = (l1 << LOGM) + s1;
#pragma unroll
    for (int c1 = 0; c1 < A; c1++) a[c1] = mb_load(src + ((size_t)k10 << LOGM) + c1 * T, in_lane, in_lane + c1);
    fill_twiddles<LA, LB, LC>(tw, aux_tw);
    const unsigned jh = t / Cn, c3 = t % Cn;
    const unsigned j1s = t / Bn, j2s = t % Bn;
    reg_ntt_dif<LA, INV>(a);
    __syncthreads();
    fp z[2][Bn];
#pragma unroll
    for (int h = 0; h < 2; h++) {
#pragma unroll
        for (int p = 0; p < A; p++) {
            const unsigned j1 = cx_brev(p, LA);
            if ((int)(j1 / AH) == h) tile[((size_t)(j1 % AH) * L2 + l1) * TP + s1] = (j1 == 0) ? a[p] : fp_mul(a[p], tw[j1 * s1]);
        }
        __syncthreads();
#pragma unroll
        for (int c2 = 0; c2 < Bn; c2++) z[h][c2] = tile[((size_t)jh * L2 + l) * TP + c2 * Cn + c3];
        __syncthreads();
    }
#pragma unroll
    for (int h = 0; h < 2; h++) {
        reg_ntt_dif<LB, INV>(z[h]);
#pragma unroll
        for (int p = 0; p < Bn; p++) {
            const unsigned j2 = cx_brev(p, LB);
            const fp v = (j2 == 0) ? z[h][p] : fp_mul(z[h][p], tw[(A * j2) * c3]);
            tile[((size_t)jh * L2 + l) * TP + j2 * Cn + (c3 ^ (j2 % Cn))] = v;
        }
        __syncthreads();
        fp x[Cn];
#pragma unroll
        for (int q = 0; q < Cn; q++) x[q] = tile[((size_t)j1s * L2 + l) * TP + j2s * Cn + (q ^ (j2s % Cn))];
        if (h == 0) __syncthreads();
        reg_ntt_dif<LC, INV>(x);
        rows_store_task<LA, LB, LC>(x, (j1s + AH * h) + A * j2s, l, log_r, post_scale, do_scale, dst + k10);
    }
}

template <int LA_, int LB_, int LC_, bool HALF_TILE_>
struct ThreeStep { static constexpr int LA = LA_, LB = LB_, LC = LC_; static constexpr bool HALF_TILE = HALF_TILE_; };
template <class F>
bool three_step_size(unsigned log_n, F &&f) {
    switch (log_n) {
    case 20: f(ThreeStep<4, 3, 3, true>{}); return true;
    case 18: f(ThreeStep<3, 3, 3, false>{}); return true;
    case 16: f(ThreeStep<3, 3, 2, false>{}); return true;
    default: return false;
    }
}

template <class S, bool INV>
hipError_t launch_three_step(const NttArgs &a, hipStream_t stream) {
    using G = V4<S::LA, S::LB, S::LC>;
    if (!a.aux || (a.prescale && !a.aux_ps)) return hipErrorInvalidValue;
    constexpr int HALVES = S::HALF_TILE ? 2 : 1;
    const size_t lds_cols = ((size_t)G::M / HALVES * L2 + G::M) * sizeof(fp);
    const size_t lds_rows = ((size_t)G::A / HALVES * L2 * (G::T + 4) + G::M) * sizeof(fp);
    const dim3 grid_cols((unsigned)G::M / L2, a.batch, a.width), grid_rows(a.batch, (unsigned)G::M / L2, a.width);
    const fp *aux_ps = a.prescale ? a.aux_ps : nullptr;
    hipError_t e;
    if constexpr (S::HALF_TILE) {
        const auto k_cols = k_ntt_cols_v5<S::LA, S::LB, S::LC, INV>;
        const auto k_rows = k_ntt_rows_v5<S::LA, S::LB, S::LC, INV>;
        if ((e = hipFuncSetAttribute((const void *)k_rows, hipFuncAttributeMaxDynamicSharedMemorySize, (int)lds_rows)) != hipSuccess) return e;
        if ((e = hipFuncSetAttribute((const void *)k_cols, hipFuncAttributeMaxDynamicSharedMemorySize, (int)lds_cols)) != hipSuccess) return e;
        hipLaunchKernelGGL(k_cols, grid_cols, dim3(G::NT), lds_cols, stream, a.in, a.scratch, a.log_n, a.in_batch_stride, a.scratch_batch_stride, a.aux,
                           aux_ps, a.aux_ps_batch_stride);
        hipLaunchKernelGGL(k_rows, grid_rows, dim3(G::NT), lds_rows, stream, (const fp *)a.scratch, a.out, a.log_n, a.post_scale, a.do_scale ? 1 : 0,
                           a.scratch_batch_stride, a.out_batch_stride, a.aux + G::M);
    } else {
        const auto k_cols = k_ntt_cols_v4<S::LA, S::LB, S::LC, INV>;
        const auto k_rows = k_ntt_rows_v4<S::LA, S::LB, S::LC, INV>;
        if ((e = hipFuncSetAttribute((const void *)k_rows, hipFuncAttributeMaxDynamicSharedMemorySize, (int)lds_rows)) != hipSuccess) return e;
        if ((e = hipFuncSetAttribute((const void *)k_cols, hipFuncAttributeMaxDynamicSharedMemorySize, (int)lds_cols)) != hipSuccess) return e;
        hipLaunchKernelGGL(k_cols, grid_cols, dim3(G::NT), lds_cols, stream, a.in, a.scratch, a.log_n, a.w, a.prescale, a.in_batch_stride,
                           a.scratch_batch_stride, a.prescale_batch_stride, a.aux, aux_ps, a.aux_ps_batch_stride);
        hipLaunchKernelGGL(k_rows, grid_rows, dim3(G::NT), lds_rows, stream, (const fp *)a.scratch, a.out, a.log_n, a.w, a.post_scale, a.do_scale ? 1 : 0,
                           a.scratch_batch_stride, a.out_batch_stride, a.aux + G::M);
    }
    return hipGetLastError();
}

constexpr int CHUNK = 16;
__global__ void k_power_table(fp *table, size_t n, fp base) {
    const size_t t = blockIdx.x * (size_t)blockDim.x + threadIdx.x;
    const size_t e0 = t * CHUNK;
    if (e0 >= n) return;
    fp x = fp_pow(base, e0);
    for (int i = 0; i < CHUNK && e0 + i < n; i++) { table[e0 + i] = x; x = fp_mul(x, base); }
}

template <int L>
hipError_t launch(const NttArgs &a, hipStream_t stream) {
    const unsigned log_r = (a.log_n + 1) / 2, log_c = a.log_n - log_r;
    const unsigned R = 1u << log_r, C = 1u << log_c;
    const size_t lds_a = ((size_t)R * L + R / 2) * sizeof(fp), lds_b = ((size_t)C * L + C / 2) * sizeof(fp);
    hipError_t e;
    if ((e = hipFuncSetAttribute((const void *)k_ntt_cols<L>, hipFuncAttributeMaxDynamicSharedMemorySize, (int)lds_a)) != hipSuccess) return e;
    if ((e = hipFuncSetAttribute((const void *)k_ntt_rows<L>, hipFuncAttributeMaxDynamicSharedMemorySize, (int)lds_b)) != hipSuccess) return e;
    hipLaunchKernelGGL(k_ntt_cols<L>, dim3(C / L, a.width, a.batch), dim3(NT), lds_a, stream, a.in, a.scratch, a.log_n, log_r, a.w, a.prescale,
                       a.in_batch_stride, a.scratch_batch_stride, a.prescale_batch_stride);
    hipLaunchKernelGGL(k_ntt_rows<L>, dim3(R / L, a.width, a.batch), dim3(NT), lds_b, stream, (const fp *)a.scratch, a.out, a.log_n, log_r, a.w,
                       a.post_scale, a.do_scale ? 1 : 0, a.scratch_batch_stride, a.out_batch_stride);
    return hipGetLastError();
}

}

__global__ void k_split_columns(const fp *__restrict__ h, fp *__restrict__ out, size_t n, unsigned log_b, fp ginv) {
    const size_t q = blockIdx.x * (size_t)blockDim.x + threadIdx.x;
    if (q >= n) return;
    const unsigned b = 1u << log_b;
    fp s = fp_pow(ginv, (uint64_t)q << log_b);
    for (unsigned i = 0; i < b; i++) {
        out[(size_t)i * n + q] = fp_mul(h[((size_t)q << log_b) + i], s);
        s = fp_mul(s, ginv);
    }
}
hipError_t split_columns(const fp *d_h, fp *d_out, unsigned log_n, unsigned log_b, fp ginv, hipStream_t stream) {
    const size_t n = (size_t)1 << log_n;
    hipLaunchKernelGGL(k_split_columns, dim3((unsigned)((n + 255) / 256)), dim3(256), 0, stream, d_h, d_out, n, log_b, ginv);
    return hipGetLastError();
}
__global__ void k_interleave_cosets(const fp *__restrict__ in, fp *__restrict__ out, size_t n, unsigned log_b) {
    const size_t i = blockIdx.x * (size_t)blockDim.x + threadIdx.x;
    if (i >= (n << log_b)) return;
    const size_t k = i & ((1u << log_b) - 1), j = i >> log_b;
    out[i] = in[k * n + j];
}
hipError_t interleave_cosets(const fp *d_in, fp *d_out, unsigned log_n, unsigned log_b, hipStream_t stream) {
    const size_t N = (size_t)1 << (log_n + log_b);
    hipLaunchKernelGGL(k_interleave_cosets, dim3((unsigned)((N + 255) / 256)), dim3(256), 0, stream, d_in, d_out, (size_t)1 << log_n, log_b);
    return hipGetLastError();
}

template <int LOGB>
__global__ __launch_bounds__(256) void k_coset_combine(const fp *__restrict__ in, fp *__restrict__ out, size_t n, const fp *__restrict__ winv, fp b_inv) {
    constexpr int B = 1 << LOGB;
    const size_t q = blockIdx.x * (size_t)256 + threadIdx.x;
    if (q >= n) return;
    in += (size_t)blockIdx.y * B * n;
    out += (size_t)blockIdx.y * B * n;
    fp v[B], wb[B];
#pragma unroll
    for (int k = 0; k < B; k++) {
        wb[k] = winv[(size_t)k * n];
        const fp x = in[(size_t)k * n + q];
        v[k] = k == 0 ? fp_mul(x, b_inv) : fp_mul(fp_mul(x, b_inv), winv[(size_t)k * q]);
    }
#pragma unroll
    for (int i = 0; i < B; i++) {
        Acc128 a = acc_zero();
#pragma unroll
        for (int k = 0; k < B; k++) {
            acc_mad(a, v[k], wb[(k * i) & (B - 1)]);
            if (k == 6) acc_fold(a);
        }
        acc_fold(a);
        out[(size_t)i * n + q] = acc_reduce(a);
    }
}
// ... 74 lines not shown
            if (kc == 0 && raw && (int)fam == d.raw_family) raw[((size_t)set * terms + t) * n + qs] = fp_mul(s, w8n[qs]);
            acc[kc] = fp_add(acc[kc], fp_mul(s, tm.c[kc][wrapped ? 1 : 0]));
        }
    }
#pragma unroll
    for (int kc = 0; kc < 4; kc++) out[(((size_t)kc * gridDim.z + set) * d.families + fam) * n + q] = acc[kc];
}
CosetMergeTerm coset_merge_term(unsigned table, uint64_t e, unsigned log_n, uint64_t base, unsigned k0) {
    CosetMergeTerm t{};
    const uint64_t n = 1ull << log_n, dq = e >> log_n, w8 = host::root_of_unity(3);
    t.table = table;
    t.r = (uint32_t)(e & (n - 1));
    const uint64_t be = host::pow(base, e);
    for (unsigned i = 0; i < 4; i++) {
        const uint64_t k = k0 + 2 * i;
        t.c[i][0] = host::mul(be, host::pow(w8, (k * (dq & 7)) & 7));
        t.c[i][1] = host::mul(t.c[i][0], host::pow(w8, k & 7));
    }
    return t;
}
hipError_t coset_even_to_odd_merged(const fp *d_b, fp *d_out, unsigned log_n, unsigned sets, const CosetMergeDesc &desc, const fp *d_winv_4n,
                                    const fp *d_w_8n, fp quarter, fp *d_raw, hipStream_t stream) {
    const size_t n = (size_t)1 << log_n;
    if (desc.families == 0 || desc.families > (unsigned)COSET_MERGE_MAX_FAMILIES || sets == 0) return hipErrorInvalidValue;
    for (unsigned f = 0; f < desc.families; f++) {
        if (desc.terms[f] == 0 || desc.terms[f] > (unsigned)COSET_MERGE_MAX_TERMS) return hipErrorInvalidValue;
        for (unsigned t = 0; t < desc.terms[f]; t++)
            if (desc.term[f][t].table >= desc.tables_per_set || desc.term[f][t].r >= n) return hipErrorInvalidValue;
    }
    if (desc.raw_family >= (int)desc.families) return hipErrorInvalidValue;
    hipLaunchKernelGGL(k_coset_even_to_odd_merged, dim3((unsigned)((n + 255) / 256), desc.families, sets), dim3(256), 0, stream, d_b, d_out, n, desc,
                       d_winv_4n, d_w_8n, quarter, d_raw);
    return hipGetLastError();
}
hipError_t coset_combine(const fp *d_b, fp *d_h, unsigned log_n, unsigned log_b, const fp *d_winv_N, fp b_inv, hipStream_t stream, unsigned tables) {
    const size_t n = (size_t)1 << log_n;
    const dim3 grid((unsigned)((n + 255) / 256), tables), block(256);
    if (log_b == 1) hipLaunchKernelGGL(k_coset_combine<1>, grid, block, 0, stream, d_b, d_h, n, d_winv_N, b_inv);
    else if (log_b == 2) hipLaunchKernelGGL(k_coset_combine<2>, grid, block, 0, stream, d_b, d_h, n, d_winv_N, b_inv);
    else if (log_b == 3) hipLaunchKernelGGL(k_coset_combine<3>, grid, block, 0, stream, d_b, d_h, n, d_winv_N, b_inv);
    else return hipErrorInvalidValue;
    return hipGetLastError();
}

bool ntt_three_step_shape(unsigned log_n, NttThreeStepShape *s) {
    return three_step_size(log_n, [s](auto split) {
        using S = decltype(split);
        *s = {S::LA + S::LB + S::LC, S::LA + S::LB + S::LC, S::LA + S::LB};
    });
}
namespace {
__global__ void k_aux_plan(fp *aux, const fp *__restrict__ w, unsigned log_r, unsigned log_c, unsigned log_kb) {
    const size_t R = (size_t)1 << log_r, C = (size_t)1 << log_c, total = R + 2 * C + (C << log_kb);
    for (size_t i = blockIdx.x * (size_t)blockDim.x + threadIdx.x; i < total; i += (size_t)gridDim.x * blockDim.x) {
        fp v;
        if (i < R) v = w[i << log_c];
        else if (i < R + C) v = w[(i - R) << log_r];
        else if (i < R + 2 * C) v = w[(i - R - C) << log_kb];
        else { const size_t q = i - R - 2 * C, kb = q >> log_c, c = q & (C - 1); v = w[kb * c]; }
        aux[i] = v;
    }
}
__global__ void k_aux_coset(fp *aux, const fp *__restrict__ w, const fp *__restrict__ s, unsigned log_r, unsigned log_c, unsigned log_kb) {
    const size_t R = (size_t)1 << log_r, C = (size_t)1 << log_c, total = R + (C << log_kb);
    for (size_t i = blockIdx.x * (size_t)blockDim.x + threadIdx.x; i < total; i += (size_t)gridDim.x * blockDim.x) {
        fp v;
        if (i < R) v = s[i << log_c];
        else { const size_t q = i - R, kb = q >> log_c, c = q & (C - 1); v = fp_mul(w[kb * c], s[c]); }
        aux[i] = v;
    }
}
}
size_t ntt_aux_plan_words(const NttThreeStepShape &s) { return ((size_t)1 << s.log_r) + ((size_t)2 << s.log_c) + ((size_t)1 << (s.log_c + s.log_kb)); }
size_t ntt_aux_coset_words(const NttThreeStepShape &s) { return ((size_t)1 << s.log_r) + ((size_t)1 << (s.log_c + s.log_kb)); }
hipError_t ntt_build_aux_plan(fp *d_aux, const fp *d_w, const NttThreeStepShape &s, hipStream_t stream) {
    hipLaunchKernelGGL(k_aux_plan, dim3(256), dim3(256), 0, stream, d_aux, d_w, s.log_r, s.log_c, s.log_kb);
    return hipGetLastError();
}
hipError_t ntt_build_aux_coset(fp *d_aux, const fp *d_w, const fp *d_s, const NttThreeStepShape &s, hipStream_t stream) {
    hipLaunchKernelGGL(k_aux_coset, dim3(256), dim3(256), 0, stream, d_aux, d_w, d_s, s.log_r, s.log_c, s.log_kb);
    return hipGetLastError();
}

hipError_t ntt_power_table(fp *d_table, size_t n, fp base, hipStream_t stream) {
    const size_t threads = (n + CHUNK - 1) / CHUNK;
    hipLaunchKernelGGL(k_power_table, dim3((unsigned)((threads + 255) / 256)), dim3(256), 0, stream, d_table, n, base);
    return hipGetLastError();
}

hipError_t ntt_columns(const NttArgs &a, hipStream_t stream) {
    if (a.log_n < NTT_MIN_LOG_N || a.log_n > NTT_MAX_LOG_N) return hipErrorInvalidValue;
    hipError_t e = hipSuccess;
    if (three_step_size(a.log_n, [&](auto split) {
            using S = decltype(split);
            e = a.inverse ? launch_three_step<S, true>(a, stream) : launch_three_step<S, false>(a, stream);
        }))
        return e;
    return (a.log_n + 1) / 2 <= 11 ? launch<8>(a, stream) : launch<4>(a, stream);
}

}
```

### certificate-stark_amd/csrc/prove.hip

```cpp
#include <hip/hip_runtime.h>
#include <string.h>
#include <algorithm>
#include <atomic>
#include <new>
#include <chrono>
#include <thread>
#include <vector>
#include "../../include/cstark.h"
#include "ctx.h"
#include "blake3.h"
#include "channel.h"
#include "deep.h"
#include "ext.h"
#include "range_batch.h"
#include "hostblake3.h"
#include "keccak.cuh"
#include "air_tx_host.h"
#include "hostfield.h"
#include "coin.h"
#include "proof_layout.h"
#include "transcript.h"

namespace cs {

// ... 76 lines not shown
constexpr int MAX_GATHER_JOBS = 32;
struct GatherBatch { GatherJob job[MAX_GATHER_JOBS]; };
__global__ void k_gather_batch(GatherBatch b) {
    const GatherJob g = b.job[blockIdx.y];
    const uint32_t q = blockIdx.x;
    if (q >= (g.dcount ? *g.dcount : g.count)) return;
    if (g.kind == 0) {
        const uint64_t *lde = (const uint64_t *)g.src;
        uint64_t *out = (uint64_t *)g.out;
        const uint32_t width = g.a, i = g.pos[q], k = lde_coset_slot(i & ((1u << g.log_b) - 1), g.log_b, g.log_s), j = i >> g.log_b;
        for (uint32_t c = threadIdx.x; c < width; c += blockDim.x) out[(size_t)q * width + c] = lde[(((size_t)k * width + c) << g.log_n) + j];
    } else {
        const uint4 *nodes = (const uint4 *)g.src;
        uint4 *out = (uint4 *)g.out;
        const uint32_t log_leaves = g.a;
        for (uint32_t t = threadIdx.x + 2 * g.lvl0; t < 2 * log_leaves; t += blockDim.x) {
            const uint32_t lvl = t >> 1, half = t & 1;
            const size_t node = ((((size_t)1 << log_leaves) + g.pos[q]) >> lvl) ^ 1;
            out[((size_t)q * log_leaves + lvl) * 2 + half] = nodes[2 * node + half];
        }
    }
}
struct GatherList {
    GatherBatch b{};
    int n = 0;
    uint32_t max_count = 0;
    void rows(const uint64_t *lde, uint32_t width, uint32_t log_n, uint32_t log_b, const uint32_t *pos, void *out, uint32_t count, uint32_t log_s = 0,
              const uint32_t *dcount = nullptr) {
        b.job[n++] = GatherJob{lde, out, pos, 0u, width, log_n, log_b, count, log_s, dcount, 0u};
        if (count > max_count) max_count = count;
    }
    void paths(const uint8_t *nodes, uint32_t log_leaves, const uint32_t *pos, void *out, uint32_t count, const uint32_t *dcount = nullptr, uint32_t lvl0 = 0) {
        b.job[n++] = GatherJob{nodes, out, pos, 1u, log_leaves, 0u, 0u, count, 0u, dcount, lvl0};
        if (count > max_count) max_count = count;
    }
    hipError_t launch(hipStream_t st) {
        if (n == 0 || max_count == 0) return hipSuccess;
        k_gather_batch<<<dim3(max_count, (unsigned)n), 128, 0, st>>>(b);
        return hipGetLastError();
    }
};
__global__ void k_gather_pub(const uint64_t *__restrict__ trace, size_t n, uint64_t *__restrict__ out, uint32_t reg0) {
    const uint32_t t = threadIdx.x;
    if (t < 14) out[t] = trace[(size_t)(reg0 + (t % 7)) * n + (t < 7 ? 0 : n - 1)];
}

template <class T>
int dev_alloc(ProveArena *a, T **p, size_t bytes) {
    HIP_TRY(hipMalloc((void **)p, bytes));
    a->owned.push_back(*p);
    return CSTARK_OK;
}

template <class T>
int arena_extra(cstark_ctx *c, ProveArena *a, size_t slot, T **p, size_t bytes) {
    if (a->extra.size() <= slot) { a->extra.resize(slot + 1, nullptr); a->extra_bytes.resize(slot + 1, 0); }
    if (a->extra[slot] && a->extra_bytes[slot] < bytes) {
        HIP_TRY(hipStreamSynchronize(c->stream));
        void *old = a->extra[slot];
        a->extra[slot] = nullptr; a->extra_bytes[slot] = 0;
        a->owned.erase(std::find(a->owned.begin(), a->owned.end(), old));
        HIP_TRY(hipFree(old));
    }
    if (!a->extra[slot]) {
        void *q;
        HIP_TRY(hipMalloc(&q, bytes));
        a->owned.push_back(q); a->extra[slot] = q; a->extra_bytes[slot] = bytes;
    }
    *p = (T *)a->extra[slot];
    return CSTARK_OK;
}

unsigned ceil_log2(uint64_t x) { unsigned l = 0; while ((1ull << l) < x) l++; return l; }

struct AirJob {
    int air = 0;
    uint32_t width = 0, log_n = 0, log_ce = 0, n_constraints = 0, n_assertions = 0, item = 0;
    std::vector<uint64_t> pub;
    std::vector<uint8_t> pub_bytes;
    int (*build)(cstark_ctx *, ProveArena *, AirJob &) = nullptr;
    int (*combine)(cstark_ctx *, ProveArena *, AirJob &, const uint64_t *ta, const uint64_t *tb, const uint64_t *ba, const uint64_t *bb, uint64_t *out) = nullptr;
    int (*combine_sets)(cstark_ctx *, ProveArena *, AirJob &, unsigned m, const uint64_t *const *ta, const uint64_t *const *tb, const uint64_t *const *ba,
                        const uint64_t *const *bb, uint64_t *const *outs) = nullptr;
    struct ColumnBatch { uint32_t col0, ncols; hipEvent_t wait[2]; };
    std::vector<ColumnBatch> batches;
    const uint64_t *pub_staging = nullptr;
    bool public_ready = false;
    bool evals_ready = false;
    uint32_t k0 = 0, nk = 8;
    bool sharded = false;
    bool dev_channel = false;
    const uint64_t *d_coefs = nullptr;
    const uint64_t *d_avalues = nullptr;
    uint32_t log_b = 3;
    uint64_t seed[7] = {};
    uint64_t number = 0;
    const uint64_t *bits = nullptr;
};

void drop_run(ProveArena *a) {
    if (a && a->run) { proof_run_free(a->run); a->run = nullptr; }
}

int get_arena(cstark_ctx *c, const AirJob &job, unsigned log_b, unsigned log_f, unsigned n_layers, size_t nq, ProveArena **out) {
    drop_run(c->arena);
    if (c->arena && c->arena->air == job.air && c->arena->log_n == job.log_n && c->arena->log_b == log_b && c->arena->log_f == log_f &&
        c->arena->layer.size() == n_layers + 1 && c->arena->open_bytes >= nq) { *out = c->arena; return CSTARK_OK; }
    if (c->arena) { HIP_TRY(hipStreamSynchronize(c->stream)); prove_arena_free(c->arena); c->arena = nullptr; }
    ProveArena *a = new (std::nothrow) ProveArena();
    if (!a) return fail(CSTARK_ERR_OOM, "host allocation failed");
    c->arena = a;
    a->air = job.air; a->log_n = job.log_n; a->log_b = log_b; a->log_f = log_f;
    const size_t n = (size_t)1 << job.log_n, b = (size_t)1 << log_b, N = n * b, W = job.width, ce = (size_t)1 << job.log_ce, f = (size_t)1 << log_f;
    RC_TRY(dev_alloc(a, &a->trace, W * n * 8));
    RC_TRY(dev_alloc(a, &a->coeffs, W * n * 8));
    RC_TRY(dev_alloc(a, &a->lde, W * N * 8));
    RC_TRY(dev_alloc(a, &a->tnodes, 2 * N * 32));
    RC_TRY(dev_alloc(a, &a->combined, N * 8));
    RC_TRY(dev_alloc(a, &a->ccoef, ce * n * 8));
    RC_TRY(dev_alloc(a, &a->clde, b * ce * n * 8));
    RC_TRY(dev_alloc(a, &a->cnodes, 2 * N * 32));
    RC_TRY(dev_alloc(a, &a->deep, N * 8));
    size_t sz = N;
    for (unsigned l = 0; l <= n_layers; l++) {
        uint64_t *e; uint8_t *t = nullptr;
        RC_TRY(dev_alloc(a, &e, sz * 8));
        if (l < n_layers) RC_TRY(dev_alloc(a, &t, 2 * (sz / f) * 32));
        a->layer.push_back(e); a->lnodes.push_back(t);
        sz /= f;
    }
    RC_TRY(dev_alloc(a, &a->d_pos, 4 * 256 * (n_layers + 2)));
    RC_TRY(dev_alloc(a, &a->d_pub, 16 * 8));
    RC_TRY(dev_alloc(a, &a->d_shifts, b * 8));
    {
        std::vector<uint64_t> sh(b);
        const uint64_t wbn = host::root_of_unity(job.log_n + log_b);
        uint64_t v = host::lde_offset();
        for (size_t k = 0; k < b; k++) { sh[k] = v; v = host::mul(v, wbn); }
        HIP_TRY(hipMemcpy(a->d_shifts, sh.data(), b * 8, hipMemcpyHostToDevice));
    }
    a->open_bytes = nq;
    const size_t log_N = job.log_n + log_b;
    const size_t per_q = W * 8 + ce * 8 + 2 * log_N * 32 + (size_t)n_layers * (f * 8 + log_N * 32);
    RC_TRY(dev_alloc(a, &a->d_open, per_q * nq + 256));
    for (hipEvent_t &e : a->ev) HIP_TRY(hipEventCreate(&e));
    *out = a;
    return CSTARK_OK;
}

int check_options(const cstark_options *opt, unsigned log_ce, unsigned *log_rem_out, unsigned *log_b_out, unsigned *log_f_out) {
    const uint32_t b = opt->blowup_factor, f = opt->fri_folding_factor;
    if (b != 2 && b != 4 && b != 8 && b != 16) return fail(CSTARK_ERR_UNSUPPORTED, "blowup_factor must be 2, 4, 8 or 16");
    if (b < (1u << log_ce)) return fail(CSTARK_ERR_INVALID_ARG, "blowup_factor below the AIR's constraint-evaluation blowup (TransactionAir / SchnorrAir 8, MerkleAir 4, RangeProofAir 2)");
    if (opt->hash_fn > 1) return fail(CSTARK_ERR_UNSUPPORTED, "hash_fn must be Blake3_256 (0) or Sha3_256 (1)");
    if (opt->field_extension > 2) return fail(CSTARK_ERR_INVALID_ARG, "field_extension must be None (0), Quadratic (1) or Cubic (2)");
    if (f != 4 && f != 8 && f != 16) return fail(CSTARK_ERR_UNSUPPORTED, "fri_folding_factor must be 4, 8 or 16");
    *log_b_out = b == 2 ? 1 : b == 4 ? 2 : b == 8 ? 3 : 4;
    *log_f_out = f == 4 ? 2 : f == 8 ? 3 : 4;
    if (opt->num_queries == 0 || opt->num_queries > 128) return fail(CSTARK_ERR_INVALID_ARG, "num_queries must be 1..128");
    if (opt->grinding_factor > 32) return fail(CSTARK_ERR_INVALID_ARG, "grinding_factor must be at most 32");
    unsigned log_rem = 0;
    while ((1u << log_rem) < opt->fri_max_remainder) log_rem++;
    if ((1u << log_rem) != opt->fri_max_remainder || log_rem < 7 || log_rem > 10) return fail(CSTARK_ERR_INVALID_ARG, "fri_max_remainder must be a power of two in 128..1024");
    *log_rem_out = log_rem;
    return CSTARK_OK;
}

// ... 12 lines not shown
    RC_TRY(grind_nonce(c, a, coin, S.opt[2], &Q.nonce));
    Q.hpos.assign(256 * (S.n_layers + 1), 0);
    transcript::draw_queries(coin, S, Q.nonce, Q.hpos.data(), Q.hpos.data() + 256, 256, Q.counts);
    HIP_TRY(hipMemcpyAsync(a->d_pos, Q.hpos.data(), Q.hpos.size() * 4, hipMemcpyHostToDevice, c->stream));
    return CSTARK_OK;
}

struct OpenBlock { size_t trows, tpaths, crows, cpaths, lrows[VMAX_LAYERS], lpaths[VMAX_LAYERS], bytes; };
OpenBlock open_block(const ProofShape &S, const uint32_t *counts, size_t start = 0, size_t align = 1) {
    OpenBlock O;
    size_t off = start;
    auto take = [&off, align](size_t bytes) { const size_t o = off; off += (bytes + align - 1) / align * align; return o; };
    O.trows = take(trace_row_bytes(S)); O.tpaths = take(path_bytes(S)); O.crows = take(comp_row_bytes(S)); O.cpaths = take(path_bytes(S));
    for (unsigned l = 0; l < S.n_layers; l++) {
        const uint32_t np = counts ? counts[l] : S.nq;
        O.lrows[l] = take(layer_row_bytes(S, np)); O.lpaths[l] = take(layer_path_bytes(S, l, np));
    }
    O.bytes = off;
    return O;
}
int host_open_block(ProveArena *a, size_t bytes) {
    if (a->h_open_bytes < bytes) {
        if (a->h_open) { HIP_TRY(hipHostFree(a->h_open)); a->h_open = nullptr; a->h_open_bytes = 0; }
        HIP_TRY(hipHostMalloc((void **)&a->h_open, bytes, hipHostMallocDefault));
        a->h_open_bytes = bytes;
    }
    return CSTARK_OK;
}
struct OpenSrc {
    const uint64_t *clde; uint64_t *const *layer; unsigned log_s;
    const uint32_t *counts, *dcount;
    const uint64_t *shard_rows; uint32_t shard_lvl0;
};
int open_stage(cstark_ctx *c, ProveArena *a, const ProofShape &S, const OpenSrc &src, uint8_t *d_block, const OpenBlock &O) {
    hipStream_t st = c->stream;
    const uint32_t nq = S.nq, W = S.width;
    GatherList gl;
    uint32_t trace_lvl0 = 0;
    if (src.shard_rows) {
        trace_lvl0 = src.shard_lvl0;
        k_split_shard_rows<<<nq, 128, 0, st>>>(src.shard_rows, W, trace_lvl0, S.log_N, (uint64_t *)(d_block + O.trows), (uint64_t *)(d_block + O.tpaths));
        HIP_TRY(hipGetLastError());
    } else gl.rows(a->lde, W, S.log_n, S.log_b, a->d_pos, d_block + O.trows, nq, src.log_s);
    gl.paths(a->tnodes, S.log_N, a->d_pos, d_block + O.tpaths, nq, nullptr, trace_lvl0);
    gl.rows(src.clde, S.ce * S.m, S.log_n, S.log_b, a->d_pos, d_block + O.crows, nq);
    gl.paths(a->cnodes, S.log_N, a->d_pos, d_block + O.cpaths, nq);
    for (unsigned l = 0; l < S.n_layers; l++) {
        const uint32_t np = src.counts ? src.counts[l] : nq, lr = layer_log_rows(S, l), *pos = a->d_pos + 256 * (l + 1), *dc = src.dcount ? src.dcount + l : nullptr;
        gl.rows(src.layer[l], S.f * S.m, lr, 0, pos, d_block + O.lrows[l], np, 0, dc);
        gl.paths(a->lnodes[l], lr, pos, d_block + O.lpaths[l], np, dc);
    }
    HIP_TRY(gl.launch(st));
    RC_TRY(host_open_block(a, O.bytes));
    HIP_TRY(hipMemcpyAsync(a->h_open, d_block, O.bytes, hipMemcpyDeviceToHost, st));
    return CSTARK_OK;
}

int lde_trace(cstark_ctx *c, ProveArena *a, const AirJob &job, uint32_t col0, uint32_t ncols) {
    const uint32_t W = job.width, log_n = job.log_n, log_b = job.log_b;
    if (job.sharded || log_b <= job.log_ce) return lde_column_range(c, a->coeffs, a->lde, W, col0, ncols, log_n, log_b, host::lde_offset(), job.k0, job.nk);
    const size_t n = (size_t)1 << log_n, ce = (size_t)1 << job.log_ce;
    const uint64_t wbn = host::root_of_unity(log_n + log_b);
    uint64_t offset = host::lde_offset();
    for (uint32_t r = 0; r < (1u << (log_b - job.log_ce)); r++) {
        RC_TRY(lde_column_range(c, a->coeffs, a->lde + (size_t)r * ce * W * n, W, col0, ncols, log_n, job.log_ce, offset, 0, (uint32_t)ce));
        offset = host::mul(offset, wbn);
    }
    return CSTARK_OK;
}
int commit_columns(cstark_ctx *c, ProveArena *a, AirJob &job, hipStream_t st, int &evi) {
    const uint32_t W = job.width, log_n = job.log_n;
    const size_t n = (size_t)1 << log_n;
    if (job.batches.empty()) {
        RC_TRY(cstark_interpolate_columns(c, a->trace, a->coeffs, W, log_n));
        HIP_TRY(hipEventRecord(a->ev[evi++], st));
        RC_TRY(lde_trace(c, a, job, 0, W));
        HIP_TRY(hipEventRecord(a->ev[evi++], st));
        return CSTARK_OK;
    }
    for (size_t i = 0; i < job.batches.size(); i++) {
        const AirJob::ColumnBatch &cb = job.batches[i];
        for (hipEvent_t e : cb.wait)
            if (e) HIP_TRY(hipStreamWaitEvent(st, e, 0));
        RC_TRY(cstark_interpolate_columns(c, a->trace + (size_t)cb.col0 * n, a->coeffs + (size_t)cb.col0 * n, cb.ncols, log_n));
        if (i + 1 == job.batches.size()) HIP_TRY(hipEventRecord(a->ev[evi++], st));
        RC_TRY(lde_trace(c, a, job, cb.col0, cb.ncols));
    }
    HIP_TRY(hipEventRecord(a->ev[evi++], st));
    return CSTARK_OK;
}

}

int grind_nonce(cstark_ctx *c, ProveArena *a, const Coin &coin, unsigned bits, uint64_t *nonce_out) {
    static const bool dev_env = [] { const char *e = getenv("CSTARK_GRIND_DEVICE"); return !e || atoi(e) != 0; }();
    if (bits == 0 || !dev_env || bits < 12) {
        *nonce_out = transcript::host_nonce(coin, bits);
        return CSTARK_OK;
    }
    unsigned long long *d_found;
    RC_TRY(arena_extra(c, a, 42, &d_found, 64));
    constexpr uint64_t CHUNK = (uint64_t)1 << 22;
    if (coin.hash_fn == 1) {
        HIP_TRY(hipMemcpyAsync(d_found + 1, coin.seed, 32, hipMemcpyHostToDevice, c->stream));
        HIP_TRY(hipMemsetAsync(d_found, 0xFF, 8, c->stream));
    }
    for (uint64_t base = 1;; base += CHUNK) {
        if (coin.hash_fn == 1) HIP_TRY(cs::grind_batch_chunk_sha3((const uint64_t *)(d_found + 1), 1, base, CHUNK, bits, d_found, c->stream));
        else HIP_TRY(cs::grind_chunk(coin.seed, base, CHUNK, bits, d_found, c->stream));
        unsigned long long found = 0;
        HIP_TRY(hipMemcpyAsync(&found, d_found, 8, hipMemcpyDeviceToHost, c->stream));
        HIP_TRY(cs::stream_wait(c->stream));
        if (found != ~0ull) { *nonce_out = found; return CSTARK_OK; }
        if (base > ((uint64_t)1 << 44)) return fail(CSTARK_ERR_HIP, "proof of work: no nonce found");
    }
}

struct ProofRun {
    cstark_options opt{};
    AirJob job;
    unsigned log_rem = 0, n_layers = 0, log_b = 3, log_f = 2, m = 1;
    ProofShape shape{};
    Coin coin;
    uint8_t trace_root[32] = {}, cons_root[32] = {}, rem_commit[32] = {};
    std::vector<uint64_t> ta[3], tb[3], ba[3], bb[3], ood_trace, ood_comp, remainder;
    std::vector<uint8_t> layer_roots;
    uint64_t *comb[3] = {}, *cco[3] = {};
    uint64_t *ccoefs = nullptr;
    uint64_t *clde = nullptr, *deep = nullptr;
    std::vector<uint64_t *> layer;
    uint8_t *d_open = nullptr;
    Queries q;
    int evi = 0, phase = 0;
    bool sharded() const { return job.sharded; }
    unsigned log_s() const { return job.sharded ? 0 : log_b - job.log_ce; }
};
void proof_run_free(ProofRun *r) { delete r; }

namespace {

int run_buffers(cstark_ctx *c, ProveArena *a, ProofRun &R) {
    const unsigned m = R.m, n_layers = R.n_layers, log_N = R.job.log_n + R.log_b;
    if (m == 1) {
        R.comb[0] = a->combined; R.cco[0] = R.ccoefs = a->ccoef; R.clde = a->clde; R.deep = a->deep; R.layer = a->layer; R.d_open = a->d_open;
        return CSTARK_OK;
    }
    const size_t b = (size_t)1 << R.log_b, N = b << R.job.log_n, W = R.job.width, CN = (size_t)1 << (R.job.log_ce + R.job.log_n), nq = R.opt.num_queries;
    const uint32_t fold = 1u << R.log_f;
    uint64_t *combined_x, *ccoef_x;
    RC_TRY(arena_extra(c, a, 16, &combined_x, 2 * CN * 8));
    RC_TRY(arena_extra(c, a, 17, &ccoef_x, 2 * CN * 8));
    RC_TRY(arena_extra(c, a, 18, &R.ccoefs, 3 * CN * 8));
    RC_TRY(arena_extra(c, a, 19, &R.clde, 3 * b * CN * 8));
    RC_TRY(arena_extra(c, a, 20, &R.deep, 3 * N * 8));
    RC_TRY(arena_extra(c, a, 21, &R.d_open, nq * (W * 8 + 192 + 2 * log_N * 32 + (size_t)n_layers * (fold * 24 + log_N * 32)) + 256));
    R.layer.resize(n_layers + 1);
    size_t sz = N;
    for (unsigned l = 0; l <= n_layers; l++) { RC_TRY(arena_extra(c, a, 22 + l, &R.layer[l], 3 * sz * 8)); sz >>= R.log_f; }
    for (unsigned q = 0; q < 3; q++) { R.comb[q] = q ? combined_x + (q - 1) * CN : a->combined; R.cco[q] = q ? ccoef_x + (q - 1) * CN : a->ccoef; }
    return CSTARK_OK;
}

int run_setup(cstark_ctx *c, const cstark_options *opt, const AirJob &job, ProofRun &R, ProveArena **a) {
    RC_TRY(check_options(opt, job.log_ce, &R.log_rem, &R.log_b, &R.log_f));
    const unsigned log_N = job.log_n + R.log_b;
    if (log_N > 24) return fail(CSTARK_ERR_UNSUPPORTED, "the LDE domain holds at most 2^24 points (2^21 trace rows at blowup 8)");
    if (job.sharded && R.log_b != 3) return fail(CSTARK_ERR_UNSUPPORTED, "sharded proofs use blowup factor 8 (one to four of its eight cosets per rank)");
    R.opt = *opt; R.job = job;
    R.job.log_b = R.log_b;
// ... 378 lines not shown
    {
        ChanStep s{};
        s.seed = d_fri; s.m = m;
        s.absorb[0].kind = CHAN_ELEMS; s.absorb[0].ptr = d_res + o_remainder; s.absorb[0].count = (uint32_t)rem_len; s.absorb[0].copy_out = d_res + o_rem;
        s.absorb[1].kind = CHAN_INT; s.absorb[1].value = 1;
        s.draw = CHAN_DRAW_QUERIES; s.count = (uint32_t)nq; s.log_domain = log_N; s.log_f = R.log_f; s.n_layers = n_layers; s.slot = 256;
        s.pos = a->d_pos; s.cnt = d_cnt;
        HIP_TRY(channel_step(s, st));
    }
    RC_TRY(open_stage(c, a, S, {R.clde, R.layer.data(), R.log_s(), nullptr, d_cnt + 1, nullptr, 0}, d_res, O));
    STAGE();
    static const bool hostprof = getenv("CSTARK_HOSTPROF") != nullptr;
    const auto hp1 = std::chrono::steady_clock::now();
    HIP_TRY(cs::stream_wait_tail(st, deep_done));
    const auto hp2 = std::chrono::steady_clock::now();
    a->timed = true; a->channel = CSTARK_CHANNEL_DEVICE;
    const uint8_t *h = a->h_open;
    const uint32_t *cnt = (const uint32_t *)(h + o_cnt);
    if (cnt[0] != nq) return fail(CSTARK_ERR_HIP, "device channel: the query positions could not be drawn");
    for (unsigned l = 0; l < n_layers; l++)
        if (cnt[l + 1] == 0 || cnt[l + 1] > nq) return fail(CSTARK_ERR_HIP, "device channel: bad folded position count");
    ProofParts p{};
    p.trace_root = h + o_troot; p.cons_root = h + o_croot; p.layer_roots = h + o_lroots; p.rem_commit = h + o_rem;
    p.ood_trace = h + o_ood; p.ood_comp = h + o_ood + ood_trace_bytes(S); p.remainder = h + o_remainder;
    p.nonce = 1;
    RC_TRY(finish_proof(S, p, h, O, cnt + 1, proof, capacity, proof_len));
    if (hostprof) {
        const auto hp3 = std::chrono::steady_clock::now();
        auto us = [](auto d) { return std::chrono::duration<double, std::micro>(d).count(); };
        fprintf(stderr, "[cstark hostprof] device channel: enqueued in %.0f us, waited %.0f us, proof written in %.0f us\n", us(hp1 - hp0), us(hp2 - hp1), us(hp3 - hp2));
    }
    return CSTARK_OK;
}
#undef STAGE
bool use_dev_channel(const cstark_options *opt, const AirJob &job) {
    static const bool host_env = [] { const char *e = getenv("CSTARK_HOST_CHANNEL"); return e && atoi(e) != 0; }();
    if (host_env || job.sharded || job.n_constraints > CSTARK_TX_NUM_CONSTRAINTS) return false;
    if (opt->hash_fn != 0 || opt->field_extension > 2 || opt->grinding_factor != 0) return false;
    uint32_t lb = 0, lf = 0, lr = 0;
    while ((1u << lb) < opt->blowup_factor && lb < 8) lb++;
    while ((1u << lf) < opt->fri_folding_factor && lf < 8) lf++;
    while ((1u << lr) < opt->fri_max_remainder && lr < 12) lr++;
    return lf >= 2 && job.log_n + lb > lr;
}

bool shard_split(uint32_t nk) {
    static const bool on = [] { const char *e = getenv("CSTARK_SHARD_SPLIT"); return !e || atoi(e) != 0; }();
    return on && (nk == 2 || nk == 4);
}
uint32_t shard_rows(uint32_t nk) { return shard_split(nk) ? nk / 2 + 4 : nk; }

int gather_roots(cstark_ctx *c, ProveArena *a, AirJob &job, uint32_t reg0 = 58) {
    const size_t n = (size_t)1 << job.log_n;
    k_gather_pub<<<1, 64, 0, c->stream>>>(a->trace, n, a->d_pub, reg0);
    HIP_TRY(hipGetLastError());
    if (job.dev_channel) return CSTARK_OK;
    job.pub.assign(14, 0);
    HIP_TRY(hipMemcpyAsync(job.pub.data(), a->d_pub, 14 * 8, hipMemcpyDeviceToHost, c->stream));
    return CSTARK_OK;
}


int tx_build(cstark_ctx *c, ProveArena *a, AirJob &job) {
    static const int mode = [] { const char *e = getenv("CSTARK_TRACE_OVERLAP"); return e ? atoi(e) : 1; }();
    if (mode == 0) {
        RC_TRY(cstark_tx_build_trace(c, a->trace));
        return gather_roots(c, a, job);
    }
    RC_TRY(tx_build_trace_split(c, a->trace));
    if (mode == 2) {
        for (hipEvent_t e : {c->ev_join, c->ev_mid, c->ev_join2}) HIP_TRY(hipStreamWaitEvent(c->stream, e, 0));
        return gather_roots(c, a, job);
    }
    const size_t n = (size_t)1 << job.log_n;
    if (!a->h_pub) HIP_TRY(hipHostMalloc((void **)&a->h_pub, 14 * 8, hipHostMallocDefault));
    k_gather_pub<<<1, 64, 0, c->side>>>(a->trace, n, a->d_pub, 58u);
    HIP_TRY(hipGetLastError());
    if (!job.dev_channel) HIP_TRY(hipMemcpyAsync(a->h_pub, a->d_pub, 14 * 8, hipMemcpyDeviceToHost, c->side));
    HIP_TRY(hipEventRecord(c->ev_join, c->side));
    job.pub_staging = a->h_pub;
    if (mode == 3)
        job.batches = {{TX_LATE_COLS, job.width - TX_LATE_COLS, {c->ev_join, c->ev_mid}}, {0, TX_LATE_COLS, {c->ev_join2, nullptr}}};
    else
        job.batches = {{TX_COPY_COLS, job.width - TX_COPY_COLS, {nullptr, nullptr}},
                       {TX_LATE_COLS, TX_COPY_COLS - TX_LATE_COLS, {c->ev_join, c->ev_mid}},
                       {0, TX_LATE_COLS, {c->ev_join2, nullptr}}};
    return CSTARK_OK;
}
int tx_combine(cstark_ctx *c, ProveArena *a, AirJob &job, const uint64_t *ta, const uint64_t *tb, const uint64_t *ba, const uint64_t *bb, uint64_t *out) {
    cstark_tx_coeffs cf;
    memcpy(cf.t_alpha, ta, sizeof cf.t_alpha); memcpy(cf.t_beta, tb, sizeof cf.t_beta);
    memcpy(cf.b_alpha, ba, sizeof cf.b_alpha); memcpy(cf.b_beta, bb, sizeof cf.b_beta);
    const uint64_t pub4[4] = {job.pub[0], job.pub[1], job.pub[7], job.pub[8]};
    uint64_t *outs[1] = {out};
    if (!job.sharded) return tx_evaluate_constraints_sets(c, a->lde, &cf, 1, pub4, outs, job.item, job.log_n, 3, 0, 8, true);
    if (shard_split(job.nk)) return tx_evaluate_constraints_shard(c, a->lde, a->coeffs, &cf, pub4, out, job.item, job.log_n, job.k0, job.nk);
    return tx_evaluate_constraints_sets(c, a->lde, &cf, 1, pub4, outs, job.item, job.log_n, 3, job.k0, job.nk, false);
}
int tx_combine_sets(cstark_ctx *c, ProveArena *a, AirJob &job, unsigned m, const uint64_t *const *ta, const uint64_t *const *tb, const uint64_t *const *ba,
                    const uint64_t *const *bb, uint64_t *const *outs) {
    cstark_tx_coeffs cf[3];
    for (unsigned q = 0; q < m; q++) {
        memcpy(cf[q].t_alpha, ta[q], sizeof cf[q].t_alpha); memcpy(cf[q].t_beta, tb[q], sizeof cf[q].t_beta);
        memcpy(cf[q].b_alpha, ba[q], sizeof cf[q].b_alpha); memcpy(cf[q].b_beta, bb[q], sizeof cf[q].b_beta);
    }
    const uint64_t pub4[4] = {job.pub[0], job.pub[1], job.pub[7], job.pub[8]};
    return tx_evaluate_constraints_sets(c, a->lde, cf, m, pub4, outs, job.item, job.log_n, 3, 0, 8, true);
}
cs::AirStageRequest air_request(ProveArena *a, const AirJob &job, const uint64_t *ta, const uint64_t *tb, const uint64_t *ba, const uint64_t *bb,
                                const uint64_t *assertion_values, uint64_t *out) {
    cs::AirStageRequest rq;
    rq.air = job.air; rq.n_items = job.air == CSTARK_AIR_SCHNORR ? job.item : 0;
    rq.log_n = job.log_n; rq.log_blowup = job.log_ce; rq.k0 = 0; rq.nk = 1u << job.log_ce;
    rq.d_lde = a->lde; rq.d_out = out;
    if (job.d_coefs) { rq.d_coefs = job.d_coefs; rq.d_avalues = job.d_avalues; }
    else { rq.t_alpha = ta; rq.t_beta = tb; rq.b_alpha = ba; rq.b_beta = bb; rq.assertion_values = assertion_values; }
    return rq;
}
int materialise_and_merge(cstark_ctx *c, ProveArena *a, AirJob &job, cs::AirStageRequest rq) {
    uint64_t *evals;
    RC_TRY(arena_extra(c, a, 0, &evals, ((size_t)rq.nk * job.n_constraints << job.log_n) * 8));
    if (!job.evals_ready) RC_TRY(cstark_air_evaluate_transitions(c, job.air, a->lde, evals, 0, job.log_n, rq.log_blowup, 0, rq.nk));
    job.evals_ready = true;
    rq.source = cs::AirTransitions::Materialised; rq.d_evals = evals;
    return air_stage(c, rq);
}
int merkle_build(cstark_ctx *c, ProveArena *a, AirJob &job) {
    RC_TRY(cstark_merkle_build_trace(c, a->trace));
    return gather_roots(c, a, job);
}
int merkle_combine(cstark_ctx *c, ProveArena *a, AirJob &job, const uint64_t *ta, const uint64_t *tb, const uint64_t *ba, const uint64_t *bb, uint64_t *out) {
    cs::AirStageRequest rq = air_request(a, job, ta, tb, ba, bb, job.pub.data(), out);
    rq.source = cs::AirTransitions::MerkleFused; rq.merkle_depth = job.item;
    return air_stage(c, rq);
}
int range_build(cstark_ctx *c, ProveArena *a, AirJob &job) {
    if (job.dev_channel) {
        const uint64_t v[3] = {job.number, 0, job.number};
        HIP_TRY(hipMemcpyAsync(a->d_pub, v, sizeof v, hipMemcpyHostToDevice, c->stream));
    }
    if (job.bits) return cstark_range_build_trace_bits(c, job.bits, job.log_n, a->trace, nullptr);
    return cstark_range_build_trace(c, job.number, a->trace);
}
int range_combine(cstark_ctx *c, ProveArena *a, AirJob &job, const uint64_t *ta, const uint64_t *tb, const uint64_t *ba, const uint64_t *bb, uint64_t *out) {
    const uint64_t vals[2] = {0, job.number};
    return materialise_and_merge(c, a, job, air_request(a, job, ta, tb, ba, bb, vals, out));
}
int rescue_build(cstark_ctx *c, ProveArena *a, AirJob &job) {
    RC_TRY(cstark_rescue_chain_build_trace(c, job.seed, job.item, a->trace));
    return gather_roots(c, a, job, 0);
}
int rescue_combine(cstark_ctx *c, ProveArena *a, AirJob &job, const uint64_t *ta, const uint64_t *tb, const uint64_t *ba, const uint64_t *bb, uint64_t *out) {
    return materialise_and_merge(c, a, job, air_request(a, job, ta, tb, ba, bb, job.pub.data(), out));
}
int schnorr_public_columns(cstark_ctx *c, ProveArena *a, AirJob &job, uint64_t **aux_lde_out, uint64_t **av_lde_out, bool compute) {
    const size_t n = (size_t)1 << job.log_n;
    uint64_t *aux, *aux_co, *aux_lde, *av_co, *av_lde;
    RC_TRY(arena_extra(c, a, 1, &aux, 19 * n * 8));
    RC_TRY(arena_extra(c, a, 2, &aux_co, 19 * n * 8));
    RC_TRY(arena_extra(c, a, 3, &aux_lde, 8 * 19 * n * 8));
    RC_TRY(arena_extra(c, a, 4, &av_co, 12 * n * 8));
    RC_TRY(arena_extra(c, a, 5, &av_lde, 8 * 12 * n * 8));
    if (compute) {
        RC_TRY(cstark_schnorr_aux_columns(c, aux));
        RC_TRY(cstark_interpolate_columns(c, aux, aux_co, 19, job.log_n));
        RC_TRY(cstark_lde_columns(c, aux_co, aux_lde, 19, job.log_n, 3, host::lde_offset(), 0, 8));
        RC_TRY(cstark_schnorr_assertion_polys(c, av_co, job.log_n));
// ... 516 lines not shown
```

### include/cstark.h

```cpp
#ifndef CSTARK_H
#define CSTARK_H
#include <stddef.h>
#include <stdint.h>

#ifdef __cplusplus
extern "C" {
#endif

typedef enum cstark_status {
    CSTARK_OK = 0,
    CSTARK_ERR_INVALID_ARG = -1,
    CSTARK_ERR_NO_DEVICE = -2,
    CSTARK_ERR_HIP = -3,
    CSTARK_ERR_OOM = -4,
    CSTARK_ERR_UNSUPPORTED = -5
} cstark_status;

typedef enum cstark_air_id {
    CSTARK_AIR_STATE_TRANSITION = 0,
    CSTARK_AIR_MERKLE_UPDATE = 1,
    CSTARK_AIR_SCHNORR = 2,
    CSTARK_AIR_RANGE = 3,
    CSTARK_AIR_RESCUE_CHAIN = 4
} cstark_air_id;

#define CSTARK_TX_TRACE_WIDTH 94
#define CSTARK_TX_CYCLE_LENGTH 1024
#define CSTARK_TX_NUM_CONSTRAINTS 115
#define CSTARK_TX_NUM_PERIODIC 48
#define CSTARK_DIGEST_BYTES 32

typedef struct cstark_tx_witness {
    uint32_t n_tx;
    uint32_t merkle_depth;
    const uint64_t *initial_roots;
    const uint64_t *final_root;
    const uint64_t *s_old_values;
    const uint64_t *r_old_values;
    const uint64_t *s_indices;
    const uint64_t *r_indices;
    const uint64_t *s_paths;
    const uint64_t *r_paths;
    const uint64_t *deltas;
    const uint64_t *sig_rx;
    const uint8_t *sig_s;
} cstark_tx_witness;

typedef struct cstark_options {
    uint32_t num_queries;
    uint32_t blowup_factor;
    uint32_t grinding_factor;
    uint32_t hash_fn;
    uint32_t field_extension;
    uint32_t fri_folding_factor;
    uint32_t fri_max_remainder;
} cstark_options;

typedef struct cstark_tx_coeffs {
    uint64_t t_alpha[CSTARK_TX_NUM_CONSTRAINTS];
    uint64_t t_beta[CSTARK_TX_NUM_CONSTRAINTS];
    uint64_t b_alpha[4];
    uint64_t b_beta[4];
} cstark_tx_coeffs;

typedef struct cstark_ctx cstark_ctx;

int cstark_ctx_create(int device, void *stream, cstark_ctx **out);
int cstark_ctx_create_own_stream(int device, cstark_ctx **out);
void cstark_ctx_destroy(cstark_ctx *ctx);
const char *cstark_last_error(void);
const char *cstark_version(void);
int cstark_ctx_synchronize(cstark_ctx *ctx);

int cstark_tx_witness_upload(cstark_ctx *ctx, const cstark_tx_witness *w);
int cstark_tx_build_trace(cstark_ctx *ctx, uint64_t *d_trace);

uint64_t cstark_field_generator(void);
uint64_t cstark_field_lde_offset(void);
uint64_t cstark_field_root_of_unity(uint32_t log_n);
int cstark_interpolate_columns(cstark_ctx *ctx, uint64_t *d_evals, uint64_t *d_coeffs, uint32_t width, uint32_t log_n);
int cstark_lde_columns(cstark_ctx *ctx, const uint64_t *d_coeffs, uint64_t *d_lde, uint32_t width, uint32_t log_n,
                       uint32_t log_blowup, uint64_t domain_offset, uint32_t k0, uint32_t nk);

int cstark_evaluate_polys_at_ext(cstark_ctx *ctx, const uint64_t *d_coeffs, uint32_t width, uint32_t log_n, uint32_t m, const uint64_t *z, uint64_t *out);
int cstark_deep_composition_ext(cstark_ctx *ctx, const uint64_t *d_trace_lde, const uint64_t *d_comp_lde, uint32_t width, uint32_t n_comp, uint32_t m,
                                const uint64_t *z, const uint64_t *ood_trace, const uint64_t *ood_comp, const uint64_t *alpha,
                                const uint64_t *beta, const uint64_t *delta, const uint64_t *deg_a, const uint64_t *deg_b, uint64_t *d_out,
                                uint32_t log_n, uint32_t log_blowup);
int cstark_fri_fold4_ext(cstark_ctx *ctx, const uint64_t *d_evals, uint64_t *d_out, uint32_t log_n, uint64_t domain_offset, uint32_t m,
                         const uint64_t *alpha);
int cstark_fri_fold_ext(cstark_ctx *ctx, const uint64_t *d_evals, uint64_t *d_out, uint32_t log_n, uint32_t folding_factor, uint64_t domain_offset,
                        uint32_t m, const uint64_t *alpha);

int cstark_hash_rows(cstark_ctx *ctx, const uint64_t *d_lde, uint8_t *d_leaves, uint32_t width,
                     uint32_t log_n, uint32_t log_blowup, uint32_t k0, uint32_t nk);
int cstark_merkle_build(cstark_ctx *ctx, uint8_t *d_nodes, uint32_t log_leaves);
int cstark_hash_rows_fn(cstark_ctx *ctx, uint32_t hash_fn, const uint64_t *d_lde, uint8_t *d_leaves, uint32_t width, uint32_t log_n,
                        uint32_t log_blowup, uint32_t k0, uint32_t nk);
int cstark_merkle_build_fn(cstark_ctx *ctx, uint32_t hash_fn, uint8_t *d_nodes, uint32_t log_leaves);

int cstark_tx_evaluate_transitions(cstark_ctx *ctx, const uint64_t *d_lde, uint64_t *d_out, uint32_t merkle_depth,
                                   uint32_t log_n, uint32_t log_blowup, uint32_t k0, uint32_t nk);
int cstark_tx_evaluate_constraints(cstark_ctx *ctx, const uint64_t *d_lde, const cstark_tx_coeffs *coeffs,
                                   const uint64_t pub_inputs[4], uint64_t *d_out, uint32_t merkle_depth,
                                   uint32_t log_n, uint32_t log_blowup, uint32_t k0, uint32_t nk);
int cstark_tx_evaluate_constraints_lde(cstark_ctx *ctx, const uint64_t *d_lde, const cstark_tx_coeffs *coeffs,
                                       const uint64_t pub_inputs[4], uint64_t *d_out, uint32_t merkle_depth, uint32_t log_n);
int cstark_tx_evaluate_constraints_ext(cstark_ctx *ctx, const uint64_t *d_lde, const cstark_tx_coeffs *coeffs, uint32_t m,
                                       const uint64_t pub_inputs[4], uint64_t *d_out, uint32_t merkle_depth,
                                       uint32_t log_n, uint32_t log_blowup, uint32_t k0, uint32_t nk);
int cstark_tx_evaluate_constraints_ext_lde(cstark_ctx *ctx, const uint64_t *d_lde, const cstark_tx_coeffs *coeffs, uint32_t m,
                                           const uint64_t pub_inputs[4], uint64_t *d_out, uint32_t merkle_depth, uint32_t log_n);
int cstark_ctx_set_part_timing(cstark_ctx *ctx, int enable);
int cstark_tx_constraint_part_ms(cstark_ctx *ctx, float *ms );
int cstark_lde_timing_ms(cstark_ctx *ctx, float *total_ms, uint64_t *elements);
int cstark_tx_constraint_degree(uint32_t i, uint32_t *base, uint32_t *cycles);
int cstark_tx_periodic_columns(uint32_t merkle_depth, uint64_t *out);

int cstark_composition_columns(cstark_ctx *ctx, const uint64_t *d_combined, uint64_t *d_cols, uint32_t log_n, uint32_t log_blowup);

int cstark_evaluate_polys_at(cstark_ctx *ctx, const uint64_t *d_coeffs, uint32_t width, uint32_t log_n, const uint64_t *points,
                             uint32_t npts, uint64_t *out);
int cstark_deep_composition(cstark_ctx *ctx, const uint64_t *d_trace_lde, const uint64_t *d_comp_lde, uint32_t width, uint32_t n_comp,
                            uint64_t z, const uint64_t *ood_trace, const uint64_t *ood_comp, const uint64_t *alpha,
                            const uint64_t *beta, const uint64_t *delta, uint64_t deg_a, uint64_t deg_b, uint64_t *d_out,
                            uint32_t log_n, uint32_t log_blowup, uint32_t k0, uint32_t nk);

int cstark_interleave_cosets(cstark_ctx *ctx, const uint64_t *d_coset_major, uint64_t *d_natural, uint32_t log_n, uint32_t log_blowup);
int cstark_fri_fold4(cstark_ctx *ctx, const uint64_t *d_evals, uint64_t *d_out, uint32_t log_n, uint64_t domain_offset, uint64_t alpha);
int cstark_fri_fold(cstark_ctx *ctx, const uint64_t *d_evals, uint64_t *d_out, uint32_t log_n, uint32_t folding_factor, uint64_t domain_offset,
                    uint64_t alpha);

#define CSTARK_PROOF_VERSION 1
#define CSTARK_PROVE_NUM_STAGES 10
int cstark_tx_prove(cstark_ctx *ctx, const cstark_options *opt, uint8_t *proof, size_t capacity, size_t *proof_len);
int cstark_air_prove(cstark_ctx *ctx, int air, const cstark_options *opt, uint64_t number, uint8_t *proof, size_t capacity, size_t *proof_len);
size_t cstark_tx_proof_size_bound(uint32_t n_tx, const cstark_options *opt);
int cstark_rescue_prove(cstark_ctx *ctx, const cstark_options *opt, const uint64_t seed[7], uint32_t chain_length, uint8_t *proof, size_t capacity,
                        size_t *proof_len);
int cstark_rescue_chain_build_trace(cstark_ctx *ctx, const uint64_t seed[7], uint32_t chain_length, uint64_t *d_trace);
int cstark_rescue_chain_periodic_columns(uint64_t *out);

uint32_t cstark_tx_shard_rows(uint32_t nk);
uint32_t cstark_tx_shard_open_words(uint32_t nk);
int cstark_tx_shard_commit(cstark_ctx *ctx, const cstark_options *opt, uint32_t k0, uint32_t nk, uint8_t *d_leaves_local);
int cstark_tx_shard_evaluate(cstark_ctx *ctx, const uint8_t *d_leaves_all, uint64_t *d_combined_local, uint32_t rows);
int cstark_tx_shard_compose(cstark_ctx *ctx, const uint64_t *d_combined_all, uint32_t total_rows, uint32_t *positions);
int cstark_tx_shard_open_rows(cstark_ctx *ctx, const uint32_t *positions, uint32_t nq, uint64_t *d_rows);
int cstark_tx_shard_finish(cstark_ctx *ctx, const uint64_t *d_rows, uint8_t *proof, size_t capacity, size_t *proof_len);
int cstark_prove_stage_ms(cstark_ctx *ctx, float *ms );
#define CSTARK_CHANNEL_HOST   0
#define CSTARK_CHANNEL_DEVICE 1
int cstark_prove_channel(cstark_ctx *ctx, uint32_t *channel);

int cstark_merkle_build_trace(cstark_ctx *ctx, uint64_t *d_trace);
int cstark_range_build_trace(cstark_ctx *ctx, uint64_t number, uint64_t *d_trace);
int cstark_range_build_trace_bits(cstark_ctx *ctx, const uint64_t *words, uint32_t log_n, uint64_t *d_trace, uint64_t *number_out);
int cstark_range_prove_bits(cstark_ctx *ctx, const cstark_options *opt, const uint64_t *words, uint32_t log_n, uint8_t *proof, size_t capacity,
                            size_t *proof_len);
int cstark_range_prove_batch(cstark_ctx *ctx, const cstark_options *opt, const uint64_t *numbers, uint32_t count, uint8_t *proofs, size_t stride,
                             size_t *lens);
int cstark_schnorr_witness_upload(cstark_ctx *ctx, uint32_t n_sig, const uint64_t *messages, const uint64_t *sig_rx, const uint8_t *sig_s);
int cstark_schnorr_build_trace(cstark_ctx *ctx, uint64_t *d_trace);
int cstark_schnorr_aux_columns(cstark_ctx *ctx, uint64_t *d_out);
int cstark_schnorr_mask_columns(uint64_t *out );
// ... 72 lines not shown
```

Baseline: 38.45.

## Add closed-form step-column interpolation and LDE for block-constant trace columns

Adds a specialised path for trace columns that stay constant within power-of-two blocks. Such a column is interpolated through a small NTT over the block values plus an elementwise product with a precomputed table. Its LDE becomes a rows-only three-step pass over a cached per-coset table scaled by those factors, skipping the full column NTT and the separate interpolation. The state-transition job now routes 27 columns with block length 1024 through this path. It relies on those columns really being block-constant, and it adds cached tables sized blowup times n.

Measured after the change: 40.22 (median of 6 runs). 1.05x the previous value.

```diff
diff --git a/certificate-stark_amd/backend.py b/certificate-stark_amd/backend.py
--- a/certificate-stark_amd/backend.py
+++ b/certificate-stark_amd/backend.py
@@ -128,6 +128,20 @@
                                           C.c_uint32(n.bit_length() - 1), C.c_uint32(log_blowup), C.c_uint64(off),
                                           C.c_uint32(k0), C.c_uint32(nk)))
         return out
+
+    def step_columns(self, evals, block_len, log_blowup, col0=0, ncols=None, offset=None, k0=0, nk=None, coeffs=None, lde=None):
+        width, n = evals.shape
+        ncols = width - col0 if ncols is None else ncols
+        nk = (1 << log_blowup) - k0 if nk is None else nk
+        if coeffs is None:
+            coeffs = self.empty_u64(width, n)
+        if lde is None:
+            lde = self.empty_u64(nk, width, n)
+        off = self.field_lde_offset() if offset is None else int(offset)
+        check(self.lib.cstark_step_columns(self.ctx, self._ptr(evals), self._ptr(coeffs), self._ptr(lde), C.c_uint32(width),
+                                           C.c_uint32(col0), C.c_uint32(ncols), C.c_uint32(n.bit_length() - 1),
+                                           C.c_uint32(block_len), C.c_uint32(log_blowup), C.c_uint64(off), C.c_uint32(k0), C.c_uint32(nk)))
+        return coeffs, lde
 
     def empty_u8(self, *shape):
         return torch.empty(shape, dtype=torch.uint8, device=self.device)
diff --git a/certificate-stark_amd/csrc/capi.hip b/certificate-stark_amd/csrc/capi.hip
--- a/certificate-stark_amd/csrc/capi.hip
+++ b/certificate-stark_amd/csrc/capi.hip
@@ -143,17 +143,21 @@
 }();
 int lde_impl_inner(cstark_ctx *c, const uint64_t *d_coeffs, uint64_t *d_lde, uint32_t width, uint32_t col0, uint32_t ncols, uint32_t log_n,
                    uint32_t log_blowup, uint64_t domain_offset, uint32_t k0, uint32_t nk);
-int lde_impl(cstark_ctx *c, const uint64_t *d_coeffs, uint64_t *d_lde, uint32_t width, uint32_t col0, uint32_t ncols, uint32_t log_n, uint32_t log_blowup,
-             uint64_t domain_offset, uint32_t k0, uint32_t nk) {
+template <class F>
+int lde_timed(cstark_ctx *c, uint64_t units, F &&run) {
     bool timed = c && c->part_timing && c->lde_ev_used + 2 <= LDE_EVENT_CAP;
     const size_t mark = timed ? c->lde_ev_used : 0;
     if (timed && lde_mark(c) != CSTARK_OK) { c->lde_ev_used = mark; timed = false; }
-    const int rc = lde_impl_inner(c, d_coeffs, d_lde, width, col0, ncols, log_n, log_blowup, domain_offset, k0, nk);
+    const int rc = run();
     if (timed) {
-        if (rc == CSTARK_OK && lde_mark(c) == CSTARK_OK) c->lde_units += (uint64_t)ncols * nk << log_n;
+        if (rc == CSTARK_OK && lde_mark(c) == CSTARK_OK) c->lde_units += units;
         else c->lde_ev_used = mark;
     }
     return rc;
+}
+int lde_impl(cstark_ctx *c, const uint64_t *d_coeffs, uint64_t *d_lde, uint32_t width, uint32_t col0, uint32_t ncols, uint32_t log_n, uint32_t log_blowup,
+             uint64_t domain_offset, uint32_t k0, uint32_t nk) {
+    return lde_timed(c, (uint64_t)ncols * nk << log_n, [&] { return lde_impl_inner(c, d_coeffs, d_lde, width, col0, ncols, log_n, log_blowup, domain_offset, k0, nk); });
 }
 int lde_impl_inner(cstark_ctx *c, const uint64_t *d_coeffs, uint64_t *d_lde, uint32_t width, uint32_t col0, uint32_t ncols, uint32_t log_n,
                    uint32_t log_blowup, uint64_t domain_offset, uint32_t k0, uint32_t nk) {
@@ -193,6 +197,61 @@
         HIP_TRY(cs::ntt_columns(a, c->stream));
     }
     return CSTARK_OK;
+}
+
+int get_step_table(cstark_ctx *c, unsigned log_n, unsigned log_b, uint64_t offset, unsigned log_block, const cs::StepTable **out) {
+    for (const cs::StepTable &t : c->steps)
+        if (t.log_n == log_n && t.log_b == log_b && t.offset == offset && t.log_block == log_block) { *out = &t; return CSTARK_OK; }
+    const NttPlan *p;
+    const CosetTable *ct;
+    RC_TRY(get_plan(c, log_n, &p));
+    RC_TRY(get_coset_table(c, log_n, log_b, offset, &ct));
+    const size_t n = (size_t)1 << log_n, b = (size_t)1 << log_b;
+    cs::StepTable t{log_n, log_b, offset, log_block, nullptr, nullptr};
+    DevGuard g;
+    HIP_TRY(g.alloc(&t.d, n * 8));
+    HIP_TRY(g.alloc(&t.w, b * n * 8));
+    cs::NttArgs a{};
+    a.in = t.d; a.scratch = t.w; a.width = 1; a.batch = (unsigned)b; a.log_n = log_n;
+    a.w = p->w; a.aux = p->aux_w;
+    a.prescale = ct->s; a.prescale_batch_stride = n;
+    a.aux_ps = ct->aux; a.aux_ps_batch_stride = ct->aux_words;
+    a.in_batch_stride = 0; a.scratch_batch_stride = n;
+    HIP_TRY(cs::ntt_step_build_tables(t.d, log_block, p->winv, a, c->stream));
+    c->steps.push_back(t);
+    g.release();
+    *out = &c->steps.back();
+    return CSTARK_OK;
+}
+int step_impl(cstark_ctx *c, uint64_t *d_evals, uint64_t *d_coeffs, uint64_t *d_lde, uint32_t width, uint32_t col0, uint32_t ncols, uint32_t log_n,
+              uint32_t block_len, uint32_t log_blowup, uint64_t domain_offset, uint32_t k0, uint32_t nk) {
+    if (!c || !d_evals || !d_coeffs || !d_lde || width == 0 || ncols == 0 || (uint64_t)col0 + ncols > width)
+        return fail(CSTARK_ERR_INVALID_ARG, "cstark_step_columns: bad argument");
+    if (log_n < cs::NTT_MIN_LOG_N || log_n > cs::NTT_MAX_LOG_N || log_blowup > 6) return fail(CSTARK_ERR_UNSUPPORTED, "unsupported domain size");
+    if (block_len == 0 || (block_len & (block_len - 1)) || block_len > (1u << log_n)) return fail(CSTARK_ERR_INVALID_ARG, "the block length must be a power of two up to the trace length");
+    if (domain_offset == 0 || domain_offset >= cs::host::P) return fail(CSTARK_ERR_INVALID_ARG, "domain offset must be a nonzero field element");
+    if ((uint64_t)k0 + nk > (1ull << log_blowup)) return fail(CSTARK_ERR_INVALID_ARG, "coset range exceeds the blowup factor");
+    const size_t n = (size_t)1 << log_n;
+    const unsigned log_block = (unsigned)__builtin_ctz(block_len);
+    if (!cs::ntt_step_shape(log_n, log_block)) {
+        RC_TRY(interpolate_impl(c, d_evals + (size_t)col0 * n, d_coeffs + (size_t)col0 * n, ncols, log_n));
+        return lde_impl(c, d_coeffs, d_lde, width, col0, ncols, log_n, log_blowup, domain_offset, k0, nk);
+    }
+    HIP_TRY(hipSetDevice(c->device));
+    const NttPlan *p;
+    const cs::StepTable *t;
+    RC_TRY(get_plan(c, log_n, &p));
+    RC_TRY(get_step_table(c, log_n, log_blowup, domain_offset, log_block, &t));
+    RC_TRY(ensure_ws(c, ((size_t)ncols << (log_n - log_block)) * 8));
+    uint64_t *fac = (uint64_t *)c->ws;
+    HIP_TRY(cs::ntt_step_coefficients(d_evals + (size_t)col0 * n, fac, d_coeffs + (size_t)col0 * n, t->d, ncols, log_n, log_block, p->winv, p->n_inv, c->stream));
+    return lde_timed(c, (uint64_t)ncols * nk << log_n, [&] {
+        cs::NttArgs a{};
+        a.out = d_lde + (size_t)col0 * n; a.width = ncols; a.batch = nk; a.log_n = log_n;
+        a.out_batch_stride = (size_t)width * n; a.aux = p->aux_w;
+        HIP_TRY(cs::ntt_step_rows(a, t->w + (size_t)k0 * n, fac, log_block, c->stream));
+        return (int)CSTARK_OK;
+    });
 }
 
 int extend_periodic_columns(cstark_ctx *c, const std::vector<uint64_t> &cols, uint32_t ncols, uint32_t log_cycle, unsigned log_n, unsigned log_b,
@@ -377,6 +436,7 @@
     if (c->coef_ev) (void)hipEventDestroy(c->coef_ev);
     for (NttPlan &p : c->plans) { (void)hipFree(p.w); (void)hipFree(p.winv); (void)hipFree(p.aux_w); (void)hipFree(p.aux_winv); }
     for (CosetTable &t : c->cosets) { (void)hipFree(t.s); (void)hipFree(t.aux); }
+    for (cs::StepTable &t : c->steps) { (void)hipFree(t.d); (void)hipFree(t.w); }
     for (PeriodicTable &t : c->periodic) { (void)hipFree(t.tab); (void)hipFree(t.coset); (void)hipFree(t.binv); }
     for (PeriodicTable &t : c->small_periodic) (void)hipFree(t.tab);
     for (cs::AssertInverseTable &t : c->assert_inv) (void)hipFree(t.tab);
@@ -491,6 +551,10 @@
                        uint64_t domain_offset, uint32_t k0, uint32_t nk) {
     return lde_impl(c, d_coeffs, d_lde, width, 0, width, log_n, log_blowup, domain_offset, k0, nk);
 }
+int cstark_step_columns(cstark_ctx *c, uint64_t *d_evals, uint64_t *d_coeffs, uint64_t *d_lde, uint32_t width, uint32_t col0, uint32_t ncols,
+                        uint32_t log_n, uint32_t block_len, uint32_t log_blowup, uint64_t domain_offset, uint32_t k0, uint32_t nk) {
+    return step_impl(c, d_evals, d_coeffs, d_lde, width, col0, ncols, log_n, block_len, log_blowup, domain_offset, k0, nk);
+}
 
 int cstark_composition_columns(cstark_ctx *c, const uint64_t *d_combined, uint64_t *d_cols, uint32_t log_n, uint32_t log_blowup) {
     if (!c || !d_combined || !d_cols) return fail(CSTARK_ERR_INVALID_ARG, "cstark_composition_columns: null argument");
@@ -880,6 +944,10 @@
 int lde_column_range(cstark_ctx *c, const uint64_t *d_coeffs, uint64_t *d_lde, uint32_t width, uint32_t col0, uint32_t ncols, uint32_t log_n,
                      uint32_t log_blowup, uint64_t domain_offset, uint32_t k0, uint32_t nk) {
     return lde_impl(c, d_coeffs, d_lde, width, col0, ncols, log_n, log_blowup, domain_offset, k0, nk);
+}
+int step_column_range(cstark_ctx *c, uint64_t *d_evals, uint64_t *d_coeffs, uint64_t *d_lde, uint32_t width, uint32_t col0, uint32_t ncols, uint32_t log_n,
+                      uint32_t block_len, uint32_t log_blowup, uint64_t domain_offset, uint32_t k0, uint32_t nk) {
+    return step_impl(c, d_evals, d_coeffs, d_lde, width, col0, ncols, log_n, block_len, log_blowup, domain_offset, k0, nk);
 }
 int tx_build_trace_split(cstark_ctx *c, uint64_t *d_trace) {
     if (!c || !d_trace) return fail(CSTARK_ERR_INVALID_ARG, "tx_build_trace_split: null argument");
diff --git a/certificate-stark_amd/csrc/ctx.h b/certificate-stark_amd/csrc/ctx.h
--- a/certificate-stark_amd/csrc/ctx.h
+++ b/certificate-stark_amd/csrc/ctx.h
@@ -74,6 +74,13 @@
     uint64_t *aux = nullptr;
     size_t aux_words = 0;
 };
+struct StepTable {
+    unsigned log_n, log_b;
+    uint64_t offset;
+    unsigned log_block;
+    uint64_t *d;
+    uint64_t *w;
+};
 struct PeriodicTable {
     unsigned depth, log_n, log_b;
     uint64_t *tab;
@@ -132,6 +139,7 @@
     cs::TxWitnessDev wit{};
     std::deque<cs::NttPlan> plans;
     std::deque<cs::CosetTable> cosets;
+    std::deque<cs::StepTable> steps;
     std::deque<cs::PeriodicTable> periodic;
     uint64_t *coef_buf = nullptr;
     void *coef_stage = nullptr;
@@ -184,9 +192,12 @@
 int tx_shard_combine(cstark_ctx *c, const uint64_t *d_parts, uint64_t *d_out, uint32_t log_n, uint32_t nk);
 constexpr uint32_t TX_LATE_COLS = 37;
 constexpr uint32_t TX_COPY_COLS = 65;
+constexpr uint32_t TX_STEP_COLS = 27;
 int tx_build_trace_split(cstark_ctx *c, uint64_t *d_trace);
 int lde_column_range(cstark_ctx *c, const uint64_t *d_coeffs, uint64_t *d_lde, uint32_t width, uint32_t col0, uint32_t ncols, uint32_t log_n,
                      uint32_t log_blowup, uint64_t domain_offset, uint32_t k0, uint32_t nk);
+int step_column_range(cstark_ctx *c, uint64_t *d_evals, uint64_t *d_coeffs, uint64_t *d_lde, uint32_t width, uint32_t col0, uint32_t ncols, uint32_t log_n,
+                      uint32_t block_len, uint32_t log_blowup, uint64_t domain_offset, uint32_t k0, uint32_t nk);
 int evaluate_ood_frames(cstark_ctx *c, const uint64_t *d_coeffs, uint32_t width, const uint64_t *d_ccoef, uint32_t n_comp, uint32_t log_n,
                         const uint64_t zpts[2], uint64_t zb, uint64_t *out_trace, uint64_t *out_comp);
 int ood_frames_dev(cstark_ctx *c, const uint64_t *d_coeffs, uint32_t width, const uint64_t *d_ccoef, uint32_t n_comp, uint32_t log_n, const uint64_t *d_pts,
diff --git a/certificate-stark_amd/csrc/ntt.h b/certificate-stark_amd/csrc/ntt.h
--- a/certificate-stark_amd/csrc/ntt.h
+++ b/certificate-stark_amd/csrc/ntt.h
@@ -31,6 +31,12 @@
 hipError_t ntt_build_aux_coset(uint64_t *d_aux, const uint64_t *d_w, const uint64_t *d_s, const NttThreeStepShape &s, hipStream_t stream);
 
 hipError_t ntt_columns(const NttArgs &a, hipStream_t stream);
+
+bool ntt_step_shape(unsigned log_n, unsigned log_block);
+hipError_t ntt_step_build_tables(uint64_t *d_d, unsigned log_block, const uint64_t *d_winv, const NttArgs &a, hipStream_t stream);
+hipError_t ntt_step_coefficients(const uint64_t *d_evals, uint64_t *d_fac, uint64_t *d_coeffs, const uint64_t *d_d, unsigned ncols, unsigned log_n,
+                                 unsigned log_block, const uint64_t *d_winv, uint64_t n_inv, hipStream_t stream);
+hipError_t ntt_step_rows(const NttArgs &a, const uint64_t *d_wtab, const uint64_t *d_fac, unsigned log_block, hipStream_t stream);
 hipError_t ntt_power_table(uint64_t *d_table, size_t n, uint64_t base, hipStream_t stream);
 
 hipError_t interleave_cosets(const uint64_t *d_in, uint64_t *d_out, unsigned log_n, unsigned log_b, hipStream_t stream);
diff --git a/certificate-stark_amd/csrc/ntt.hip b/certificate-stark_amd/csrc/ntt.hip
--- a/certificate-stark_amd/csrc/ntt.hip
+++ b/certificate-stark_amd/csrc/ntt.hip
@@ -227,6 +227,16 @@
     }
 }
 
+template <int LA, int LB, int LC>
+__device__ __forceinline__ void rows_load_step(fp (&a)[1 << LA], const fp *__restrict__ rows, unsigned in_lane, unsigned s1, const fp *__restrict__ fac,
+                                               unsigned fac_mask) {
+    constexpr int A = V4<LA, LB, LC>::A, T = V4<LA, LB, LC>::T;
+#pragma unroll
+    for (int c1 = 0; c1 < A; c1++) a[c1] = mb_load(rows + c1 * T, in_lane, in_lane + c1);
+#pragma unroll
+    for (int c1 = 0; c1 < A; c1++) a[c1] = fp_mul(a[c1], fac[(c1 * T + s1) & fac_mask]);
+}
+
 constexpr int V4_TILES = 1;
 
 
@@ -437,6 +447,64 @@
             }
         }
         __syncthreads();
+    }
+}
+
+template <int LA, int LB, int LC>
+__global__ __launch_bounds__((V4<LA, LB, LC>::NT), 4) void k_ntt_rows_step_v4(const fp *__restrict__ wtab, const fp *__restrict__ fac, fp *__restrict__ out,
+                                                                             unsigned log_n, unsigned log_t, size_t out_batch_stride,
+                                                                             const fp *__restrict__ aux_tw) {
+    using G = V4<LA, LB, LC>;
+    constexpr int A = G::A, Bn = G::Bn, Cn = G::Cn, T = G::T, LOGM = G::LOGM;
+    constexpr int TP = T + 4;
+    extern __shared__ __attribute__((aligned(16))) fp smem[];
+    fp *tile = smem;
+    fp *tw = smem + (size_t)A * L2 * TP;
+    const unsigned log_r = log_n - LOGM;
+    const size_t n = (size_t)1 << log_n;
+    const fp *src = wtab + blockIdx.x * n;
+    fp *dst = out + blockIdx.x * out_batch_stride + (size_t)blockIdx.z * n;
+    const unsigned s1 = threadIdx.x % T, l1 = threadIdx.x / T;
+    const unsigned l = threadIdx.x % L2, t = threadIdx.x / L2;
+    const unsigned k10 = xcd_pair_tile(blockIdx.y) * L2;
+    fp a[A];
+    rows_load_step<LA, LB, LC>(a, src + ((size_t)k10 << LOGM), (l1 << LOGM) + s1, s1, fac + ((size_t)blockIdx.z << log_t), (1u << log_t) - 1);
+    fill_twiddles<LA, LB, LC>(tw, aux_tw);
+    reg_ntt_dif<LA, false>(a);
+    __syncthreads();
+#pragma unroll
+    for (int p = 0; p < A; p++) {
+        const unsigned j1 = cx_brev(p, LA);
+        tile[((size_t)j1 * L2 + l1) * TP + s1] = (j1 == 0) ? a[p] : fp_mul(a[p], tw[j1 * s1]);
+    }
+    __syncthreads();
+    fp z[G::J2][Bn];
+#pragma unroll
+    for (int j = 0; j < G::J2; j++) {
+        const unsigned u = t + T * j, j1 = u / Cn, c3 = u % Cn;
+#pragma unroll
+        for (int c2 = 0; c2 < Bn; c2++) z[j][c2] = tile[((size_t)j1 * L2 + l) * TP + c2 * Cn + c3];
+    }
+    __syncthreads();
+#pragma unroll
+    for (int j = 0; j < G::J2; j++) {
+        const unsigned u = t + T * j, j1 = u / Cn, c3 = u % Cn;
+        reg_ntt_dif<LB, false>(z[j]);
+#pragma unroll
+        for (int p = 0; p < Bn; p++) {
+            const unsigned j2 = cx_brev(p, LB);
+            tile[((size_t)j1 * L2 + l) * TP + j2 * Cn + (c3 ^ (j2 % Cn))] = (j2 == 0) ? z[j][p] : fp_mul(z[j][p], tw[(A * j2) * c3]);
+        }
+    }
+    __syncthreads();
+#pragma unroll
+    for (int j = 0; j < G::J3; j++) {
+        const unsigned v = t + T * j, j1 = v / Bn, j2 = v % Bn;
+        fp x[Cn];
+#pragma unroll
+        for (int c3 = 0; c3 < Cn; c3++) x[c3] = tile[((size_t)j1 * L2 + l) * TP + j2 * Cn + (c3 ^ (j2 % Cn))];
+        reg_ntt_dif<LC, false>(x);
+        rows_store_task<LA, LB, LC>(x, j1 + A * j2, l, log_r, 0, 0, dst + k10);
     }
 }
 
@@ -560,6 +628,64 @@
     }
 }
 
+template <int LA, int LB, int LC>
+__global__ __launch_bounds__((V4<LA, LB, LC>::NT), V5_ROWS_WAVES) void k_ntt_rows_step_v5(const fp *__restrict__ wtab, const fp *__restrict__ fac,
+                                                                                         fp *__restrict__ out, unsigned log_n, unsigned log_t,
+                                                                                         size_t out_batch_stride, const fp *__restrict__ aux_tw) {
+    constexpr bool INV = false;
+    using G = V4<LA, LB, LC>;
+    constexpr int A = G::A, Bn = G::Bn, Cn = G::Cn, T = G::T, LOGM = G::LOGM, AH = A / 2;
+    static_assert(G::J2 == 2 && G::J3 == 2 && Bn == AH && Cn == AH, "two tasks per thread and step, one per half");
+    constexpr int TP = T + 4;
+    extern __shared__ __attribute__((aligned(16))) fp smem[];
+    fp *tile = smem;
+    fp *tw = smem + (size_t)AH * L2 * TP;
+    const unsigned log_r = log_n - LOGM;
+    const size_t n = (size_t)1 << log_n;
+    const fp *src = wtab + blockIdx.x * n;
+    fp *dst = out + blockIdx.x * out_batch_stride + (size_t)blockIdx.z * n;
+    const unsigned s1 = threadIdx.x % T, l1 = threadIdx.x / T;
+    const unsigned l = threadIdx.x % L2, t = threadIdx.x / L2;
+    const unsigned k10 = xcd_pair_tile(blockIdx.y) * L2;
+    fp a[A];
+    rows_load_step<LA, LB, LC>(a, src + ((size_t)k10 << LOGM), (l1 << LOGM) + s1, s1, fac + ((size_t)blockIdx.z << log_t), (1u << log_t) - 1);
+    fill_twiddles<LA, LB, LC>(tw, aux_tw);
+    const unsigned jh = t / Cn, c3 = t % Cn;
+    const unsigned j1s = t / Bn, j2s = t % Bn;
+    reg_ntt_dif<LA, INV>(a);
+    __syncthreads();
+    fp z[2][Bn];
+#pragma unroll
+    for (int h = 0; h < 2; h++) {
+#pragma unroll
+        for (int p = 0; p < A; p++) {
+            const unsigned j1 = cx_brev(p, LA);
+            if ((int)(j1 / AH) == h) tile[((size_t)(j1 % AH) * L2 + l1) * TP + s1] = (j1 == 0) ? a[p] : fp_mul(a[p], tw[j1 * s1]);
+        }
+        __syncthreads();
+#pragma unroll
+        for (int c2 = 0; c2 < Bn; c2++) z[h][c2] = tile[((size_t)jh * L2 + l) * TP + c2 * Cn + c3];
+        __syncthreads();
+    }
+#pragma unroll
+    for (int h = 0; h < 2; h++) {
+        reg_ntt_dif<LB, INV>(z[h]);
+#pragma unroll
+        for (int p = 0; p < Bn; p++) {
+            const unsigned j2 = cx_brev(p, LB);
+            const fp v = (j2 == 0) ? z[h][p] : fp_mul(z[h][p], tw[(A * j2) * c3]);
+            tile[((size_t)jh * L2 + l) * TP + j2 * Cn + (c3 ^ (j2 % Cn))] = v;
+        }
+        __syncthreads();
+        fp x[Cn];
+#pragma unroll
+        for (int q = 0; q < Cn; q++) x[q] = tile[((size_t)j1s * L2 + l) * TP + j2s * Cn + (q ^ (j2s % Cn))];
+        if (h == 0) __syncthreads();
+        reg_ntt_dif<LC, INV>(x);
+        rows_store_task<LA, LB, LC>(x, (j1s + AH * h) + A * j2s, l, log_r, 0, 0, dst + k10);
+    }
+}
+
 template <int LA_, int LB_, int LC_, bool HALF_TILE_>
 struct ThreeStep { static constexpr int LA = LA_, LB = LB_, LC = LC_; static constexpr bool HALF_TILE = HALF_TILE_; };
 template <class F>
@@ -572,10 +698,12 @@
     }
 }
 
+struct StepPass { const fp *wtab, *fac; unsigned log_t; };
 template <class S, bool INV>
-hipError_t launch_three_step(const NttArgs &a, hipStream_t stream) {
+hipError_t launch_three_step(const NttArgs &a, hipStream_t stream, const StepPass *step = nullptr) {
     using G = V4<S::LA, S::LB, S::LC>;
-    if (!a.aux || (a.prescale && !a.aux_ps)) return hipErrorInvalidValue;
+    if (!a.aux || (a.prescale && !a.aux_ps) || (step && INV)) return hipErrorInvalidValue;
+    const bool do_cols = !step || !step->wtab, do_rows = !step;
     constexpr int HALVES = S::HALF_TILE ? 2 : 1;
     const size_t lds_cols = ((size_t)G::M / HALVES * L2 + G::M) * sizeof(fp);
     const size_t lds_rows = ((size_t)G::A / HALVES * L2 * (G::T + 4) + G::M) * sizeof(fp);
@@ -587,19 +715,39 @@
         const auto k_rows = k_ntt_rows_v5<S::LA, S::LB, S::LC, INV>;
         if ((e = hipFuncSetAttribute((const void *)k_rows, hipFuncAttributeMaxDynamicSharedMemorySize, (int)lds_rows)) != hipSuccess) return e;
         if ((e = hipFuncSetAttribute((const void *)k_cols, hipFuncAttributeMaxDynamicSharedMemorySize, (int)lds_cols)) != hipSuccess) return e;
-        hipLaunchKernelGGL(k_cols, grid_cols, dim3(G::NT), lds_cols, stream, a.in, a.scratch, a.log_n, a.in_batch_stride, a.scratch_batch_stride, a.aux,
-                           aux_ps, a.aux_ps_batch_stride);
-        hipLaunchKernelGGL(k_rows, grid_rows, dim3(G::NT), lds_rows, stream, (const fp *)a.scratch, a.out, a.log_n, a.post_scale, a.do_scale ? 1 : 0,
-                           a.scratch_batch_stride, a.out_batch_stride, a.aux + G::M);
+        if (do_cols)
+            hipLaunchKernelGGL(k_cols, grid_cols, dim3(G::NT), lds_cols, stream, a.in, a.scratch, a.log_n, a.in_batch_stride, a.scratch_batch_stride, a.aux,
+                               aux_ps, a.aux_ps_batch_stride);
+        if (do_rows)
+            hipLaunchKernelGGL(k_rows, grid_rows, dim3(G::NT), lds_rows, stream, (const fp *)a.scratch, a.out, a.log_n, a.post_scale, a.do_scale ? 1 : 0,
+                               a.scratch_batch_stride, a.out_batch_stride, a.aux + G::M);
+        if constexpr (!INV) {
+            if (step && step->wtab) {
+                const auto k_step = k_ntt_rows_step_v5<S::LA, S::LB, S::LC>;
+                if ((e = hipFuncSetAttribute((const void *)k_step, hipFuncAttributeMaxDynamicSharedMemorySize, (int)lds_rows)) != hipSuccess) return e;
+                hipLaunchKernelGGL(k_step, grid_rows, dim3(G::NT), lds_rows, stream, step->wtab, step->fac, a.out, a.log_n, step->log_t, a.out_batch_stride,
+                                   a.aux + G::M);
+            }
+        }
     } else {
         const auto k_cols = k_ntt_cols_v4<S::LA, S::LB, S::LC, INV>;
         const auto k_rows = k_ntt_rows_v4<S::LA, S::LB, S::LC, INV>;
         if ((e = hipFuncSetAttribute((const void *)k_rows, hipFuncAttributeMaxDynamicSharedMemorySize, (int)lds_rows)) != hipSuccess) return e;
         if ((e = hipFuncSetAttribute((const void *)k_cols, hipFuncAttributeMaxDynamicSharedMemorySize, (int)lds_cols)) != hipSuccess) return e;
-        hipLaunchKernelGGL(k_cols, grid_cols, dim3(G::NT), lds_cols, stream, a.in, a.scratch, a.log_n, a.w, a.prescale, a.in_batch_stride,
-                           a.scratch_batch_stride, a.prescale_batch_stride, a.aux, aux_ps, a.aux_ps_batch_stride);
-        hipLaunchKernelGGL(k_rows, grid_rows, dim3(G::NT), lds_rows, stream, (const fp *)a.scratch, a.out, a.log_n, a.w, a.post_scale, a.do_scale ? 1 : 0,
-                           a.scratch_batch_stride, a.out_batch_stride, a.aux + G::M);
+        if (do_cols)
+            hipLaunchKernelGGL(k_cols, grid_cols, dim3(G::NT), lds_cols, stream, a.in, a.scratch, a.log_n, a.w, a.prescale, a.in_batch_stride,
+                               a.scratch_batch_stride, a.prescale_batch_stride, a.aux, aux_ps, a.aux_ps_batch_stride);
+        if (do_rows)
+            hipLaunchKernelGGL(k_rows, grid_rows, dim3(G::NT), lds_rows, stream, (const fp *)a.scratch, a.out, a.log_n, a.w, a.post_scale, a.do_scale ? 1 : 0,
+                               a.scratch_batch_stride, a.out_batch_stride, a.aux + G::M);
+        if constexpr (!INV) {
+            if (step && step->wtab) {
+                const auto k_step = k_ntt_rows_step_v4<S::LA, S::LB, S::LC>;
+                if ((e = hipFuncSetAttribute((const void *)k_step, hipFuncAttributeMaxDynamicSharedMemorySize, (int)lds_rows)) != hipSuccess) return e;
+                hipLaunchKernelGGL(k_step, grid_rows, dim3(G::NT), lds_rows, stream, step->wtab, step->fac, a.out, a.log_n, step->log_t, a.out_batch_stride,
+                                   a.aux + G::M);
+            }
+        }
     }
     return hipGetLastError();
 }
@@ -840,6 +988,64 @@
     return hipGetLastError();
 }
 
+bool ntt_step_shape(unsigned log_n, unsigned log_block) {
+    NttThreeStepShape s;
+    return log_block < log_n && ntt_three_step_shape(log_n, &s) && log_n - log_block <= s.log_c;
+}
+namespace {
+__global__ __launch_bounds__(256) void k_step_d(fp *__restrict__ d, const fp *__restrict__ winv, size_t n, unsigned log_t) {
+    const size_t k = blockIdx.x * (size_t)256 + threadIdx.x;
+    if (k >= n) return;
+    d[k] = k == 0 ? FP_ONE : (k & (((size_t)1 << log_t) - 1)) == 0 ? 0 : fp_inv(fp_sub(winv[k], FP_ONE));
+}
+__global__ __launch_bounds__(NT) void k_step_factors(const fp *__restrict__ evals, fp *__restrict__ fac, unsigned log_n, unsigned log_t,
+                                                     const fp *__restrict__ winv, fp n_inv, fp t_inv) {
+    extern __shared__ __attribute__((aligned(16))) fp smem[];
+    const unsigned T = 1u << log_t, log_block = log_n - log_t;
+    fp *tile = smem, *tw = smem + T;
+    const fp *col = evals + ((size_t)blockIdx.x << log_n);
+    for (unsigned t = threadIdx.x; t < T; t += NT) tile[t] = col[(size_t)t << log_block];
+    for (unsigned e = threadIdx.x; e < T / 2; e += NT) tw[e] = winv[(size_t)e << log_block];
+    __syncthreads();
+    lds_ntt_dif<1>(tile, log_t, tw);
+    for (unsigned j = threadIdx.x; j < T; j += NT) {
+        const fp g = tile[bitrev(j, log_t)];
+        fac[((size_t)blockIdx.x << log_t) + j] = j == 0 ? fp_mul(g, t_inv) : fp_mul(fp_mul(g, n_inv), fp_sub(winv[(size_t)j << log_block], FP_ONE));
+    }
+}
+__global__ __launch_bounds__(256) void k_step_coeffs(const fp *__restrict__ fac, const fp *__restrict__ d, fp *__restrict__ coeffs, unsigned log_n,
+                                                     unsigned log_t) {
+    const size_t k = blockIdx.x * (size_t)256 + threadIdx.x;
+    coeffs[((size_t)blockIdx.y << log_n) + k] = fp_mul(fac[((size_t)blockIdx.y << log_t) + (k & (((size_t)1 << log_t) - 1))], d[k]);
+}
+}
+hipError_t ntt_step_build_tables(uint64_t *d_d, unsigned log_block, const uint64_t *d_winv, const NttArgs &a, hipStream_t stream) {
+    if (!ntt_step_shape(a.log_n, log_block) || a.inverse || a.width != 1 || a.in != d_d) return hipErrorInvalidValue;
+    const size_t n = (size_t)1 << a.log_n;
+    hipLaunchKernelGGL(k_step_d, dim3((unsigned)(n / 256)), dim3(256), 0, stream, d_d, d_winv, n, a.log_n - log_block);
+    const StepPass columns_only{nullptr, nullptr, 0};
+    hipError_t e = hipErrorInvalidValue;
+    three_step_size(a.log_n, [&](auto split) { e = launch_three_step<decltype(split), false>(a, stream, &columns_only); });
+    return e;
+}
+hipError_t ntt_step_coefficients(const uint64_t *d_evals, uint64_t *d_fac, uint64_t *d_coeffs, const uint64_t *d_d, unsigned ncols, unsigned log_n,
+                                 unsigned log_block, const uint64_t *d_winv, uint64_t n_inv, hipStream_t stream) {
+    if (!ntt_step_shape(log_n, log_block) || ncols == 0 || ncols > 65535) return hipErrorInvalidValue;
+    const unsigned log_t = log_n - log_block;
+    const uint64_t t_inv = host::inv(host::from_u64((uint64_t)1 << log_t));
+    hipLaunchKernelGGL(k_step_factors, dim3(ncols), dim3(NT), (size_t)3 * 8 << (log_t - 1), stream, d_evals, d_fac, log_n, log_t, d_winv, n_inv, t_inv);
+    hipLaunchKernelGGL(k_step_coeffs, dim3((unsigned)(((size_t)1 << log_n) / 256), ncols), dim3(256), 0, stream, (const fp *)d_fac, d_d, d_coeffs, log_n,
+                       log_t);
+    return hipGetLastError();
+}
+hipError_t ntt_step_rows(const NttArgs &a, const uint64_t *d_wtab, const uint64_t *d_fac, unsigned log_block, hipStream_t stream) {
+    if (!ntt_step_shape(a.log_n, log_block) || a.inverse || !d_wtab || !d_fac) return hipErrorInvalidValue;
+    const StepPass rows{d_wtab, d_fac, a.log_n - log_block};
+    hipError_t e = hipErrorInvalidValue;
+    three_step_size(a.log_n, [&](auto split) { e = launch_three_step<decltype(split), false>(a, stream, &rows); });
+    return e;
+}
+
 hipError_t ntt_power_table(fp *d_table, size_t n, fp base, hipStream_t stream) {
     const size_t threads = (n + CHUNK - 1) / CHUNK;
     hipLaunchKernelGGL(k_power_table, dim3((unsigned)((threads + 255) / 256)), dim3(256), 0, stream, d_table, n, base);
diff --git a/certificate-stark_amd/csrc/prove.hip b/certificate-stark_amd/csrc/prove.hip
--- a/certificate-stark_amd/csrc/prove.hip
+++ b/certificate-stark_amd/csrc/prove.hip
@@ -182,7 +182,7 @@
     int (*combine)(cstark_ctx *, ProveArena *, AirJob &, const uint64_t *ta, const uint64_t *tb, const uint64_t *ba, const uint64_t *bb, uint64_t *out) = nullptr;
     int (*combine_sets)(cstark_ctx *, ProveArena *, AirJob &, unsigned m, const uint64_t *const *ta, const uint64_t *const *tb, const uint64_t *const *ba,
                         const uint64_t *const *bb, uint64_t *const *outs) = nullptr;
-    struct ColumnBatch { uint32_t col0, ncols; hipEvent_t wait[2]; };
+    struct ColumnBatch { uint32_t col0, ncols; hipEvent_t wait[2]; uint32_t block = 0; };
     std::vector<ColumnBatch> batches;
     const uint64_t *pub_staging = nullptr;
     bool public_ready = false;
@@ -361,9 +361,11 @@
         const AirJob::ColumnBatch &cb = job.batches[i];
         for (hipEvent_t e : cb.wait)
             if (e) HIP_TRY(hipStreamWaitEvent(st, e, 0));
-        RC_TRY(cstark_interpolate_columns(c, a->trace + (size_t)cb.col0 * n, a->coeffs + (size_t)cb.col0 * n, cb.ncols, log_n));
+        const bool step = cb.block != 0 && !job.sharded && job.log_b <= job.log_ce;
+        if (!step) RC_TRY(cstark_interpolate_columns(c, a->trace + (size_t)cb.col0 * n, a->coeffs + (size_t)cb.col0 * n, cb.ncols, log_n));
         if (i + 1 == job.batches.size()) HIP_TRY(hipEventRecord(a->ev[evi++], st));
-        RC_TRY(lde_trace(c, a, job, cb.col0, cb.ncols));
+        if (step) RC_TRY(step_column_range(c, a->trace, a->coeffs, a->lde, W, cb.col0, cb.ncols, log_n, cb.block, job.log_b, host::lde_offset(), job.k0, job.nk));
+        else RC_TRY(lde_trace(c, a, job, cb.col0, cb.ncols));
     }
     HIP_TRY(hipEventRecord(a->ev[evi++], st));
     return CSTARK_OK;
@@ -908,7 +910,8 @@
     if (mode == 3)
         job.batches = {{TX_LATE_COLS, job.width - TX_LATE_COLS, {c->ev_join, c->ev_mid}}, {0, TX_LATE_COLS, {c->ev_join2, nullptr}}};
     else
-        job.batches = {{TX_COPY_COLS, job.width - TX_COPY_COLS, {nullptr, nullptr}},
+        job.batches = {{TX_COPY_COLS, TX_STEP_COLS, {nullptr, nullptr}, 1024},
+                       {TX_COPY_COLS + TX_STEP_COLS, job.width - TX_COPY_COLS - TX_STEP_COLS, {nullptr, nullptr}},
                        {TX_LATE_COLS, TX_COPY_COLS - TX_LATE_COLS, {c->ev_join, c->ev_mid}},
                        {0, TX_LATE_COLS, {c->ev_join2, nullptr}}};
     return CSTARK_OK;
diff --git a/include/cstark.h b/include/cstark.h
--- a/include/cstark.h
+++ b/include/cstark.h
@@ -81,6 +81,8 @@
 int cstark_interpolate_columns(cstark_ctx *ctx, uint64_t *d_evals, uint64_t *d_coeffs, uint32_t width, uint32_t log_n);
 int cstark_lde_columns(cstark_ctx *ctx, const uint64_t *d_coeffs, uint64_t *d_lde, uint32_t width, uint32_t log_n,
                        uint32_t log_blowup, uint64_t domain_offset, uint32_t k0, uint32_t nk);
+int cstark_step_columns(cstark_ctx *ctx, uint64_t *d_evals, uint64_t *d_coeffs, uint64_t *d_lde, uint32_t width, uint32_t col0, uint32_t ncols,
+                        uint32_t log_n, uint32_t block_len, uint32_t log_blowup, uint64_t domain_offset, uint32_t k0, uint32_t nk);
 
 int cstark_evaluate_polys_at_ext(cstark_ctx *ctx, const uint64_t *d_coeffs, uint32_t width, uint32_t log_n, uint32_t m, const uint64_t *z, uint64_t *out);
 int cstark_deep_composition_ext(cstark_ctx *ctx, const uint64_t *d_trace_lde, const uint64_t *d_comp_lde, uint32_t width, uint32_t n_comp, uint32_t m,
```
